# apache/paimon

Measured on NVIDIA H100. Metric: merged rows/sec at 16 runs x 40M rows, higher is better.
Workload: dtype int64

## Files before the change

### paimon_b200/csrc/api.cu

```cuda
#include <algorithm>
#include <cstdlib>
#include <cstring>
#include <map>
#include <memory>
#include <mutex>
#include <queue>

#include "pg_internal.h"

namespace pg {

static thread_local std::string g_last_error;
void set_error(const std::string &msg) { g_last_error = msg; }
pg_status fail(pg_status code, const std::string &msg) {
    g_last_error = msg;
    return code;
}

static int g_device = -1;

struct Arena {
    unsigned char *base = nullptr;
    size_t cap = 0, top = 0;
    cudaError_t reserve(size_t bytes) {
        top = 0;
        if (bytes <= cap) return cudaSuccess;
        if (base) cudaFree(base);
        base = nullptr;
        cap = 0;
        cudaError_t e = cudaMalloc((void **)&base, bytes);
        if (e == cudaSuccess) cap = bytes;
        return e;
    }
    void *take(size_t bytes) {
        size_t a = align256(top);
        if (a + bytes > cap) return nullptr;
        top = a + bytes;
        return base + a;
    }
    void release() {
        if (base) cudaFree(base);
        base = nullptr;
        cap = top = 0;
    }
    ~Arena() { release(); }
};

struct Merge {
    std::shared_ptr<const Spec> spec;
    std::vector<std::shared_ptr<const Run>> runs;
    std::vector<std::weak_ptr<const Run>> bound;
    std::vector<int64_t> row0;
    int k = 0;
    int64_t n_in = 0;
    size_t desc_cap = 0;
    cudaStream_t stream = nullptr;
    cudaEvent_t ev[5] = {nullptr, nullptr, nullptr, nullptr, nullptr};
    std::vector<int64_t> varlen_bound;
    KeyDesc key{};
    SeqFields seq{};
    MergeFlags flags{};
    std::vector<ColDesc> cols;
    std::vector<int32_t> varlen_cols;
    std::vector<uint8_t> emit;
    void *d_desc = nullptr;
    const void **d_key_ptrs = nullptr;
    const int32_t **d_key_offs = nullptr;
    const int64_t **d_seq_ptrs = nullptr;
    const int8_t **d_kind_ptrs = nullptr;
    ColPtrs d_ptrs{};
    int64_t *d_run_rows = nullptr;
    ColDesc *d_cols = nullptr;
    int32_t *d_tile_counter = nullptr;
    int32_t *d_col_order = nullptr;
    int32_t *d_varlen_cols = nullptr;
    int n_passes = 0;
    const SeqGroups *d_groups = nullptr;
    bool has_group_aggs = false;
    pg_out_column *d_out_cols = nullptr;
    int64_t *d_totals = nullptr;
    int32_t *d_err = nullptr;
    int64_t *h_totals = nullptr;
    int32_t *h_err = nullptr;
    std::vector<pg_out_column> out_cols;
    Arena work;
    Arena outbuf;
    int64_t n_out = 0;
    bool has_batch = false;
    pg_stats stats{};
    ~Merge() {
        if (g_device >= 0) cudaSetDevice(g_device);
        if (stream) cudaStreamSynchronize(stream);
        if (d_desc) cudaFree(d_desc);
        if (h_totals) cudaFreeHost(h_totals);
        for (cudaEvent_t e : ev) if (e) cudaEventDestroy(e);
        if (stream) cudaStreamDestroy(stream);
    }
};


Table<Schema> g_schemas(1);
static Table<Spec> g_specs(2);
Table<Run> g_runs(3);
static Table<Merge> g_merges(4);

pg_status ensure_device() {
    if (g_device < 0) return fail(PG_ERR_INVALID, "pg_init has not been called");
    PG_CUDA(cudaSetDevice(g_device));
    return PG_OK;
}

static pg_status copy_batch(std::vector<void *> &dsts, std::vector<void *> &srcs, std::vector<size_t> &sizes,
                            cudaMemcpyKind kind, cudaStream_t stream) {
    if (dsts.empty()) return PG_OK;
    static bool batch_ok = true;
    if (batch_ok && dsts.size() > 1) {
        cudaMemcpyAttributes attr{};
        attr.srcAccessOrder = cudaMemcpySrcAccessOrderStream;
        size_t attr_idx = 0, fail_idx = 0;
        cudaError_t e = cudaMemcpyBatchAsync(dsts.data(), srcs.data(), sizes.data(), dsts.size(), &attr, &attr_idx, 1,
                                             &fail_idx, stream);
        if (e == cudaSuccess) return PG_OK;
        cudaGetLastError();
        batch_ok = false;
    }
    for (size_t i = 0; i < dsts.size(); i++) PG_CUDA(cudaMemcpyAsync(dsts[i], srcs[i], sizes[i], kind, stream));
    return PG_OK;
}
static std::mutex g_buf_mu;
static std::multimap<size_t, void *> g_free_bufs;
static size_t g_free_bytes = 0;
static size_t buf_cache_limit() {
    static size_t lim = [] {
        const char *e = getenv("PG_RUN_CACHE_BYTES");
        return e ? (size_t)strtoull(e, nullptr, 10) : ((size_t)16 << 30);
    }();
    return lim;
}
static void buf_trim(size_t keep_bytes) {
    std::vector<void *> drop;
    {
        std::lock_guard<std::mutex> g(g_buf_mu);
        while (g_free_bytes > keep_bytes && !g_free_bufs.empty()) {
            auto it = std::prev(g_free_bufs.end());
            drop.push_back(it->second);
            g_free_bytes -= it->first;
            g_free_bufs.erase(it);
        }
    }
    for (void *p : drop) cudaFree(p);
}
void *buf_take(size_t bytes, size_t *got) {
    {
        std::lock_guard<std::mutex> g(g_buf_mu);
        auto it = g_free_bufs.lower_bound(bytes);
        if (it != g_free_bufs.end() && it->first <= bytes + bytes / 2 + (1 << 20)) {
            void *p = it->second;
            *got = it->first;
            g_free_bytes -= it->first;
            g_free_bufs.erase(it);
            return p;
        }
    }
    void *p = nullptr;
    if (cudaMalloc(&p, bytes) != cudaSuccess) {
        cudaGetLastError();
        buf_trim(0);
        if (cudaMalloc(&p, bytes) != cudaSuccess) return nullptr;
    }
    *got = bytes;
    return p;
}
void buf_give(void *p, size_t bytes) {
    {
        std::lock_guard<std::mutex> g(g_buf_mu);
        if (g_free_bytes + bytes <= buf_cache_limit()) {
            g_free_bufs.emplace(bytes, p);
            g_free_bytes += bytes;
            return;
        }
    }
    cudaFree(p);
}
cudaStream_t copy_stream() {
    static thread_local cudaStream_t st = nullptr;
    if (!st) cudaStreamCreateWithFlags(&st, cudaStreamNonBlocking);
    return st;
}

pg_status batch_columns(uint64_t handle, BatchColumns *out) {
    if (std::shared_ptr<Merge> m = g_merges.get(handle)) {
        if (!m->has_batch) return fail(PG_ERR_INVALID, "no batch: call pg_merge_execute first");
        if (m->stream) PG_CUDA(cudaStreamSynchronize(m->stream));
        out->schema = m->spec->schema;
        out->n_rows = m->n_out;
        for (const pg_out_column &oc : m->out_cols) out->cols.push_back(DevColumn{oc.data, oc.offsets, oc.validity});
        out->merge = std::move(m);
        return PG_OK;
    }
    std::shared_ptr<Run> r = g_runs.get(handle);
    if (!r) return fail(PG_ERR_INVALID, "unknown run / merge handle");
    out->schema = r->schema;
    out->n_rows = r->n_rows;
    out->cols = r->cols;
    out->run = std::move(r);
    return PG_OK;
}


pg_status oom(const char *who, const char *what, size_t bytes) {
    size_t fr = 0, tot = 0;
    cudaMemGetInfo(&fr, &tot);
    cudaGetLastError();
    return fail(PG_ERR_CUDA, std::string(who) + ": out of device memory for " + what + " (" + std::to_string(bytes >> 20) +
                                 " MiB wanted, " + std::to_string(fr >> 20) + " of " + std::to_string(tot >> 20) + " MiB free)");
}

pg_status check_file_desc(const pg_file_desc &f) {
    if (f.mem != PG_MEM_HOST && f.mem != PG_MEM_DEVICE)
        return fail(PG_ERR_INVALID, "file descriptor: memory kind " + std::to_string(f.mem) + " is neither host nor device");
    if (f.size < 0) return fail(PG_ERR_INVALID, "file descriptor: negative size");
    if (f.size > 0 && !f.bytes) return fail(PG_ERR_INVALID, "file descriptor: no bytes for a file of " + std::to_string(f.size) + " bytes");
    return PG_OK;
}

pg_status check_section_args(uint64_t schema, const pg_file_desc *files, int n_files, int n_runs, const uint64_t *out_runs,
                             std::shared_ptr<const Schema> *s) {
    *s = g_schemas.get(schema);
    if (!*s || !out_runs || n_files < 0 || n_runs < 0 || (n_files > 0 && !files))
        return fail(PG_ERR_INVALID, "bad schema handle or null argument");
    for (int i = 0; i < n_files; i++) {
        pg_status st = check_file_desc(files[i]);
        if (st) return st;
        if (files[i].run < 0 || files[i].run >= n_runs)
            return fail(PG_ERR_INVALID, "file descriptor: run index " + std::to_string(files[i].run) + " out of range");
    }
    return PG_OK;
}

pg_status file_image(Scratch &scratch, const uint8_t *bytes, int64_t size, const char *who, const uint8_t **out) {
    uint8_t *d = (uint8_t *)scratch.take((size_t)size + 64);
    if (!d) return oom(who, "a file image", (size_t)size);
    PG_CUDA(cudaMemcpyAsync(d, bytes, (size_t)size, cudaMemcpyHostToDevice, scratch.stream));
    *out = d;
    return PG_OK;
}

pg_status RunBuilder::read_columns(const uint8_t *read_cols, const char *const *column_names) {
    names = column_names;
    if (names)
        for (int c = 0; c < nc; c++)
            if (!names[c]) return fail(PG_ERR_INVALID, std::string(who) + ": column name " + std::to_string(c) + " is NULL");
    if (!read_cols) return PG_OK;
    for (int c = 0; c < schema->n_key + 2; c++)
        if (!read_cols[c]) return fail(PG_ERR_INVALID, std::string(who) + ": key, sequence number and kind columns are always read");
    for (int c = 0; c < nc; c++) read[c] = read_cols[c] != 0;
    return PG_OK;
}

pg_status RunBuilder::add_file(int run, int64_t rows, const std::vector<std::string> &cols) {
    if (!names && (int)cols.size() != nc)
        return fail(PG_ERR_UNSUPPORTED, std::string(who) + ": the file has " + std::to_string(cols.size()) + " columns and the "
                                        "read schema " + std::to_string(nc) + " (pass the field names)");
    std::unordered_map<std::string, int> by_name;
    if (names) for (int i = 0; i < (int)cols.size(); i++) by_name.emplace(cols[i], i);
    std::vector<int> fc(nc, -2);
    for (int c = 0; c < nc; c++) {
        if (!read[c]) continue;
        fc[c] = c;
        if (names) {
            auto it = by_name.find(names[c]);
            fc[c] = it == by_name.end() ? -1 : it->second;
        }
        if (fc[c] == -1 && (c < schema->n_key + 2 || !schema->field(c).nullable))
            return fail(PG_ERR_UNSUPPORTED, std::string(who) + ": the file has no column '" + names[c] + "' and the read "
                                            "schema does not allow NULL for it");
        const size_t i = (size_t)run * nc + c;
        if (fc[c] == -1) missing[i] = 1;
        if (rows > 0) with_rows[i] |= fc[c] == -1 ? 2 : 1;
    }
    file_col.push_back(std::move(fc));
    file_row0.push_back(place_file(run, rows));
    return PG_OK;
}

pg_status RunBuilder::check_runs() const {
    for (int64_t n : run_rows)
        if (n > 0x7fffffffLL) return fail(PG_ERR_UNSUPPORTED, std::string(who) + ": more than 2^31 rows in one run");
    for (size_t i = 0; i < with_rows.size(); i++)
        if (with_rows[i] == 3 && is_varlen(schema->field((int)(i % nc)).type))
            return fail(PG_ERR_UNSUPPORTED, std::string(who) + ": a var-len column exists in some files with rows of a sorted "
                                            "run only (mixed table schemas inside one run: not decoded on device)");
    return PG_OK;
}

pg_status RunBuilder::alloc(const std::vector<uint8_t> &bitmap, const std::vector<uint8_t> &zero) {
    const int n_runs = (int)run_rows.size();
    scratch.runs.resize(n_runs);
    out.assign((size_t)n_runs * nc, OutColumn());
    for (int r = 0; r < n_runs; r++) {
        const int64_t n = run_rows[r];
        scratch.runs[r] = std::make_unique<Run>(schema, n);
        auto main_bytes = [&](int c) { const int w = type_width(schema->field(c).type); return w ? (size_t)n * w : 4 * (size_t)(n + 1); };
        const size_t vb = align256((size_t)((n + 31) / 32) * 4 + 64);
        size_t vbytes = 0;
        for (int c = 0; c < nc; c++) if (read[c] && bitmap[c]) vbytes += vb;
        size_t total = vbytes;
        std::vector<size_t> o_main(nc);
        for (int c = 0; c < nc; c++) {
            o_main[c] = total;
            if (read[c]) total += align256(main_bytes(c) + 64);
        }
        scratch.runs[r]->bufs.emplace_back(total + 256);
        unsigned char *base = scratch.runs[r]->bufs.back().get();
        if (!base) return oom(who, "the columns of a run", total);
        if (vbytes) PG_CUDA(cudaMemsetAsync(base, 0, vbytes, scratch.stream));
        size_t vt = 0;
        for (int c = 0; c < nc; c++) {
            if (!read[c]) continue;
            OutColumn &o = out[(size_t)r * nc + c];
            if (bitmap[c]) { o.validity = (uint32_t *)(base + vt); vt += vb; decoded_bytes += (n + 7) / 8; }
            if (type_width(schema->field(c).type)) o.data = base + o_main[c];
            else o.offsets = (int32_t *)(base + o_main[c]);
            decoded_bytes += (int64_t)main_bytes(c);
            if (zero[(size_t)r * nc + c]) PG_CUDA(cudaMemsetAsync(base + o_main[c], 0, main_bytes(c), scratch.stream));
        }
    }
    return PG_OK;
}

pg_status RunBuilder::alloc_payload(const std::vector<int64_t> &payload) {
    bool any = false;
    for (int c = 0; c < nc; c++) any |= read[c] && is_varlen(schema->field(c).type);
    if (!any) return PG_OK;
    for (int r = 0; r < (int)run_rows.size(); r++) {
        size_t sum = 256;
        for (int c = 0; c < nc; c++)
            if (read[c] && is_varlen(schema->field(c).type)) sum += align256((size_t)payload[(size_t)r * nc + c] + 64);
        Run &run = *scratch.runs[r];
        run.bufs.emplace_back(sum);
        unsigned char *pl = run.bufs.back().get();
        if (!pl) return oom(who, "the var-len payload of a run", sum);
        size_t pt = 0;
        for (int c = 0; c < nc; c++) {
            if (!read[c] || !is_varlen(schema->field(c).type)) continue;
            const int64_t bytes = payload[(size_t)r * nc + c];
            out[(size_t)r * nc + c].data = pl + pt;
            run.varlen_bytes[c] = bytes;
            decoded_bytes += bytes;
            pt += align256((size_t)bytes + 64);
        }
    }
    return PG_OK;
}

void RunBuilder::finish(uint64_t *out_runs, int64_t bytes_h2d, pg_section_info *info) {
    const int n_runs = (int)run_rows.size();
    for (int r = 0; r < n_runs; r++) {
        Run &run = *scratch.runs[r];
        for (int c = 0; c < nc; c++) {
            const OutColumn &o = out[(size_t)r * nc + c];
            if (read[c]) run.cols[c] = DevColumn{o.data ? o.data : run.bufs[0].get(), o.offsets, (const uint8_t *)o.validity};
        }
        run.bytes_h2d = r == 0 ? bytes_h2d : 0;
        out_runs[r] = g_runs.put(std::move(scratch.runs[r]));
    }
    if (info) {
        memset(info, 0, sizeof(*info));
        for (int64_t n : run_rows) info->n_rows += n;
        info->n_runs = n_runs;
        info->decoded_bytes = decoded_bytes;
    }
}

SectionFrame::SectionFrame(std::shared_ptr<const Schema> s, int n_runs, const char *who)
    : stream(copy_stream()), scratch(stream), b(std::move(s), n_runs, scratch, who) {}

pg_status SectionFrame::start(const uint8_t *read_cols, const char *const *names) {
    PG_CUDA(cudaEventCreate(&tm.e0));
    PG_CUDA(cudaEventCreate(&tm.e1));
    PG_CUDA(cudaEventRecord(tm.e0, stream));
    return b.read_columns(read_cols, names);
}

pg_status SectionFrame::place(const pg_file_desc *files, int n_files) {
    d_file.assign(n_files, nullptr);
    for (int f = 0; f < n_files; f++) {
        file_bytes += files[f].size;
        if (files[f].mem == PG_MEM_DEVICE) { d_file[f] = files[f].bytes; continue; }
        { pg_status st = file_image(scratch, files[f].bytes, files[f].size, b.who, &d_file[f]); if (st) return st; }
        h2d += files[f].size;
    }
    return PG_OK;
}

pg_status SectionFrame::finish(const int32_t *d_err, uint64_t *out_runs, pg_section_info *info) {
    PG_CUDA(cudaEventRecord(tm.e1, stream));
    int32_t herr = 0;
    SmallReads rb(stream);
    { pg_status rs = rb.add(&herr, d_err, 4); if (!rs) rs = rb.finish(); if (rs) return rs; }
    PG_CUDA(cudaGetLastError());
    { pg_status st = kernel_error(herr, b.who); if (st) return st; }
    b.finish(out_runs, h2d, info);
    if (info) {
        info->file_bytes = file_bytes;
        info->page_bytes = page_bytes;
        info->n_files = (int32_t)d_file.size();
        info->launches = launches;
        info->ms_decode = tm.ms();
    }
    return PG_OK;
}

static void free_outputs(Merge *m, bool release_memory = false) {
    m->out_cols.clear();
    m->has_batch = false;
    if (release_memory) {
        if (m->stream) cudaStreamSynchronize(m->stream);
        m->outbuf.release();
    }
}


static bool agg_supports_retract(int agg) {
    return agg == PG_AGG_SUM || agg == PG_AGG_PRODUCT || agg == PG_AGG_LAST_VALUE ||
           agg == PG_AGG_LAST_NON_NULL_VALUE || agg == PG_AGG_PRIMARY_KEY;
}

static pg_status build_descriptors(Merge *m) {
    const Schema *s = m->spec->schema.get();
    const Spec *sp = m->spec.get();
    if (s->n_key < 1 || s->n_key > PG_MAX_KEY_FIELDS)
        return fail(PG_ERR_UNSUPPORTED, "more than 4 primary-key fields are not implemented on the device");
    m->key = KeyDesc{};
    m->key.n_fields = s->n_key;
    int key_bytes = 0;
    bool all_fixed = true;
    for (int f = 0; f < s->n_key; f++) {
        int t = s->key_fields[f].type;
        if (t == PG_FLOAT || t == PG_DOUBLE)
            return fail(PG_ERR_UNSUPPORTED, "FLOAT / DOUBLE primary keys are not implemented on the device "
                                            "(the reference's comparator treats NaN as equal to everything)");
        m->key.type[f] = t;
        m->key.width[f] = type_width(t);
        if (is_varlen(t)) all_fixed = false;
        key_bytes += type_width(t);
    }
    m->key.exact = all_fixed && key_bytes <= 8;
    m->seq = SeqFields{};
    if (sp->seq_fields.size() > 4)
        return fail(PG_ERR_UNSUPPORTED, "more than 4 'sequence.field' columns are not implemented on the device");
    for (size_t i = 0; i < sp->seq_fields.size(); i++) {
        int vf = sp->seq_fields[i];
        if (vf < 0 || vf >= s->n_val) return fail(PG_ERR_INVALID, "sequence.field index out of range");
        int t = s->val_fields[vf].type;
        if (is_varlen(t))
            return fail(PG_ERR_UNSUPPORTED, "var-len 'sequence.field' columns are not implemented on the device");
        m->seq.col[i] = s->n_key + 2 + vf;
        m->seq.type[i] = t;
        m->seq.width[i] = type_width(t);
    }
    m->seq.n = (int32_t)sp->seq_fields.size();
    m->seq.ascending = sp->seq_ascending ? 1 : 0;
    m->flags = MergeFlags{sp->engine, sp->ignore_delete, sp->remove_record_on_delete, sp->drop_delete};

    const int nc = s->n_cols();
    m->cols.assign(nc, ColDesc{});
    m->varlen_cols.clear();
    m->emit.assign(nc, 1);
    for (int c = s->n_key + 2; c < nc; c++)
        if (!sp->read_fields.empty() && !sp->read_fields[c - s->n_key - 2]) m->emit[c] = 0;
    std::vector<uint8_t> needed = m->emit;
    for (int32_t vf : sp->seq_fields) if (vf >= 0 && vf < s->n_val) needed[s->n_key + 2 + vf] = 1;
    for (int32_t vf : sp->group_seq_fields) if (vf >= 0 && vf < s->n_val) needed[s->n_key + 2 + vf] = 1;
    for (int r = 0; r < m->k; r++)
        for (int c = 0; c < nc; c++)
            if (needed[c] && m->runs[r]->n_rows > 0 && !m->runs[r]->cols[c].data && !m->runs[r]->cols[c].offsets)
                return fail(PG_ERR_INVALID, "run " + std::to_string(r) + " has no buffers for column " + std::to_string(c) +
                                            ", which the merge reads (read-type projection dropped a field the merge "
                                            "function compares or emits)");
    for (int c = 0; c < nc; c++) {
        pg_field f = s->field(c);
        ColDesc &cd = m->cols[c];
        cd.type = f.type;
        cd.width = type_width(f.type);
        cd.nullable = f.nullable;
        cd.agg = PG_AGG_NONE;
        cd.retract = RT_OK;
        cd.varlen_index = -1;
        cd.decimal = 0;
        if (is_varlen(f.type) && m->emit[c]) {
            cd.varlen_index = (int)m->varlen_cols.size();
            m->varlen_cols.push_back(c);
        }
        if (c < s->n_key) { cd.mode = CM_KEY; cd.nullable = 0; }
        else if (c == s->n_key) { cd.mode = CM_SEQ; cd.nullable = 0; }
        else if (c == s->n_key + 1) { cd.mode = CM_KIND; cd.nullable = 0; }
        else {
            int vi = c - s->n_key - 2;
            int agg = sp->agg.empty() ? PG_AGG_NONE : sp->agg[vi];
            bool ign = !sp->ignore_retract.empty() && sp->ignore_retract[vi];
            const int32_t dec = sp->decimal.empty() ? 0 : sp->decimal[vi];
            const int32_t fold_dec = agg == PG_AGG_SUM || agg == PG_AGG_PRODUCT ? dec : 0;
            if (sp->engine == PG_ENGINE_AGGREGATE) {
                if (agg == PG_AGG_NONE) agg = PG_AGG_LAST_NON_NULL_VALUE;
                bool numeric = f.type == PG_INT8 || f.type == PG_INT16 || f.type == PG_INT32 ||
                               f.type == PG_INT64 || f.type == PG_FLOAT || f.type == PG_DOUBLE;
                if ((agg == PG_AGG_SUM || agg == PG_AGG_PRODUCT) && !numeric)
                    return fail(PG_ERR_INVALID, "sum/product need a numeric column");
                if ((agg == PG_AGG_BOOL_AND || agg == PG_AGG_BOOL_OR) && f.type != PG_BOOL)
                    return fail(PG_ERR_INVALID, "bool_and/bool_or need a BOOLEAN column");
                if ((agg == PG_AGG_MAX || agg == PG_AGG_MIN) && f.type == PG_BOOL)
                    return fail(PG_ERR_INVALID, "Incomparable type: BOOLEAN");
                if (agg < PG_AGG_SUM || agg > PG_AGG_PRIMARY_KEY)
                    return fail(PG_ERR_UNSUPPORTED, "aggregate function not implemented on the device");
                cd.mode = CM_FOLD;
                cd.agg = agg;
                cd.decimal = fold_dec;
                cd.nullable = 1;
                cd.retract = ign ? RT_IGNORE : (agg_supports_retract(agg) ? RT_OK : RT_ERROR);
            } else {
                const bool in_group = sp->n_groups() > 0 && sp->field_group[vi] >= 0;
                if (sp->engine == PG_ENGINE_PARTIAL_UPDATE && !in_group && agg != PG_AGG_NONE &&
                    agg != PG_AGG_LAST_NON_NULL_VALUE && agg != PG_AGG_PRIMARY_KEY)
                    return fail(PG_ERR_INVALID, "Must use sequence group for aggregation functions");
                cd.mode = CM_SELECT;
                if (sp->n_groups() > 0 && sp->field_group[vi] >= 0) {
                    const int g = sp->field_group[vi];
                    bool is_seq = false;
                    for (int j = sp->group_seq_start[g]; j < sp->group_seq_start[g + 1]; j++)
                        if (sp->group_seq_fields[j] == vi) is_seq = true;
                    cd.mode = is_seq ? CM_GSEQ : CM_GVAL;
                    cd.agg = g;
                    cd.nullable = 1;
                    if (!is_seq && agg != PG_AGG_NONE) {
                        cd.mode = CM_GAGG;
                        cd.agg = agg;
                        cd.decimal = fold_dec;
                        cd.group = g;
                        cd.retract = ign ? RT_IGNORE : (agg_supports_retract(agg) ? RT_OK : RT_ERROR);
                        m->has_group_aggs = true;
                    }
                }
            }
        }
    }

    const int k = m->k, nk = s->n_key, nv = (int)m->varlen_cols.size();
    size_t o_key = 0;
    size_t o_koff = o_key + align256(sizeof(void *) * k * nk);
    size_t o_seq = o_koff + align256(sizeof(void *) * k * nk);
    size_t o_kind = o_seq + align256(sizeof(void *) * k);
    size_t o_pd = o_kind + align256(sizeof(void *) * k);
    size_t o_po = o_pd + align256(sizeof(void *) * (size_t)k * nc);
    size_t o_pv = o_po + align256(sizeof(void *) * (size_t)k * nc);
    size_t o_rows = o_pv + align256(sizeof(void *) * (size_t)k * nc);
    size_t o_cols = o_rows + align256(sizeof(int64_t) * k);
    size_t o_out = o_cols + align256(sizeof(ColDesc) * nc);
    size_t o_tot = o_out + align256(sizeof(pg_out_column) * nc);
    size_t o_err = o_tot + align256(sizeof(int64_t) * (nv + 1));
    size_t o_cnt = o_err + 256;
    size_t o_ord = o_cnt + 256;
    size_t o_vlc = o_ord + align256(sizeof(int32_t) * (2 * (size_t)nc + 2));
    size_t o_sg = o_vlc + align256(sizeof(int32_t) * (size_t)(nv + 1));
    size_t total = o_sg + align256(sizeof(SeqGroups));
    std::vector<unsigned char> host(total, 0);
    m->varlen_bound.assign(nv, 0);
    for (int r = 0; r < k; r++) {
        const Run *run = m->runs[r].get();
        for (int f = 0; f < nk; f++) {
            ((const void **)(host.data() + o_key))[r * nk + f] = run->cols[f].data;
            ((const void **)(host.data() + o_koff))[r * nk + f] = run->cols[f].offsets;
        }
        ((const void **)(host.data() + o_seq))[r] = run->cols[nk].data;
        ((const void **)(host.data() + o_kind))[r] = run->cols[nk + 1].data;
        for (int c = 0; c < nc; c++) {
            ((const void **)(host.data() + o_pd))[(size_t)c * k + r] = run->cols[c].data;
            ((const void **)(host.data() + o_po))[(size_t)c * k + r] = run->cols[c].offsets;
            ((const void **)(host.data() + o_pv))[(size_t)c * k + r] = run->cols[c].validity;
            if (m->cols[c].varlen_index >= 0) m->varlen_bound[m->cols[c].varlen_index] += run->varlen_bytes[c];
        }
        ((int64_t *)(host.data() + o_rows))[r] = run->n_rows;
    }
    memcpy(host.data() + o_cols, m->cols.data(), sizeof(ColDesc) * nc);
    {
        int32_t *ord = (int32_t *)(host.data() + o_ord);
        int32_t *vlc = (int32_t *)(host.data() + o_vlc);
        int n = 0;
        for (int c = 0; c < nc; c++) if (m->emit[c] && m->cols[c].width == 0) ord[n++] = c;
        for (int c = 0; c < nc; c++) if (m->emit[c] && m->cols[c].width != 0) ord[n++] = c;
        m->n_passes = n;
        for (int v = 0; v < nv; v++) vlc[v] = m->varlen_cols[v];
    }
    m->d_groups = nullptr;
    if (sp->n_groups() > 0) {
        SeqGroups *sg = (SeqGroups *)(host.data() + o_sg);
        sg->n = sp->n_groups();
        for (int g = 0; g <= sg->n; g++) sg->start[g] = sp->group_seq_start[g];
        for (int j = 0; j < sp->group_seq_start[sg->n]; j++) {
            const int vf = sp->group_seq_fields[j];
            sg->col[j] = s->n_key + 2 + vf;
            sg->type[j] = s->val_fields[vf].type;
            sg->width[j] = type_width(s->val_fields[vf].type);
        }
        for (int g = 0; g < sg->n; g++) sg->partial_delete[g] = sp->group_partial_delete[g];
    }
    if (!m->d_desc || total > m->desc_cap) {
        if (m->d_desc) cudaFree(m->d_desc);
        m->d_desc = nullptr;
        PG_CUDA(cudaMalloc(&m->d_desc, total));
        m->desc_cap = total;
    }
    { pg_status ts = small_h2d(m->d_desc, host.data(), total, m->stream); if (ts) return ts; }
    PG_CUDA(cudaStreamSynchronize(m->stream));
    unsigned char *d = (unsigned char *)m->d_desc;
    m->d_key_ptrs = (const void **)(d + o_key);
    m->d_key_offs = (const int32_t **)(d + o_koff);
    m->d_seq_ptrs = (const int64_t **)(d + o_seq);
    m->d_kind_ptrs = (const int8_t **)(d + o_kind);
    m->d_ptrs.data = (const void *const *)(d + o_pd);
    m->d_ptrs.offsets = (const int32_t *const *)(d + o_po);
    m->d_ptrs.validity = (const uint32_t *const *)(d + o_pv);
    m->d_run_rows = (int64_t *)(d + o_rows);
    m->d_cols = (ColDesc *)(d + o_cols);
    m->d_out_cols = (pg_out_column *)(d + o_out);
    m->d_totals = (int64_t *)(d + o_tot);
    m->d_err = (int32_t *)(d + o_err);
    m->d_tile_counter = (int32_t *)(d + o_cnt);
    m->d_col_order = (int32_t *)(d + o_ord);
    m->d_varlen_cols = (int32_t *)(d + o_vlc);
    if (sp->n_groups() > 0) m->d_groups = (const SeqGroups *)(d + o_sg);
    if (!m->h_totals) PG_CUDA(cudaMallocHost((void **)&m->h_totals, sizeof(int64_t) * (nv + 1) + 16));
    m->h_err = (int32_t *)(m->h_totals + nv + 1);
    return PG_OK;
}

pg_status kernel_error(int code, const char *who) {
    static const struct { int code; pg_status st; const char *msg; } kErrors[] = {
        {KERR_PU_DELETE, PG_ERR_MERGE_FUNCTION,
         "By default, Partial update can not accept delete records, you can choose one of the "
         "following solutions:\n1. Configure 'ignore-delete' to ignore delete records.\n"
         "2. Configure 'partial-update.remove-record-on-delete' to remove the whole row when "
         "receiving delete records.\n3. Configure 'sequence-group's to retract partial columns. "
         "Also configure 'partial-update.remove-record-on-sequence-group' to remove the whole "
         "row when receiving deleted records of `specified sequence group`."},
        {KERR_FIRST_ROW_RETRACT, PG_ERR_MERGE_FUNCTION,
         "By default, First row merge engine can not accept DELETE/UPDATE_BEFORE records.\n"
         "You can config 'ignore-delete' to ignore the DELETE/UPDATE_BEFORE records."},
        {KERR_AGG_RETRACT, PG_ERR_MERGE_FUNCTION,
         "Aggregate function does not support retraction, If you allow this function to ignore "
         "retraction messages, you can configure 'fields.${field_name}.ignore-retract'='true'."},
        {KERR_DIV_ZERO, PG_ERR_MERGE_FUNCTION, "ArithmeticException: / by zero"},
        {KERR_DEC_DIV_ZERO, PG_ERR_MERGE_FUNCTION, "ArithmeticException: Division by zero"},
        {KERR_DEC_DIV_UNDEFINED, PG_ERR_MERGE_FUNCTION, "ArithmeticException: Division undefined"},
        {KERR_DEC_NON_TERMINATING, PG_ERR_MERGE_FUNCTION,
         "ArithmeticException: Non-terminating decimal expansion; no exact representable decimal result."},
        {KERR_TILE_OVERFLOW, PG_ERR_INTERNAL,
         "a merge tile overflowed (does a run contain duplicate keys? SortMergeReader.java:37 requires unique keys per reader)"},
        {KERR_OFFSET_OVERFLOW, PG_ERR_INTERNAL, "a var-len column exceeds 2 GiB of payload"},
        {KERR_BAD_PAGE, PG_ERR_FORMAT, "a page or stream does not decode (malformed file or unsupported encoding)"},
        {KERR_PQ_HEADER, PG_ERR_FORMAT, "malformed or truncated page header"},
        {KERR_PQ_NO_DICT, PG_ERR_FORMAT, "dictionary-encoded page without dictionary"},
        {KERR_PQ_ROWS, PG_ERR_FORMAT, "page row counts do not add up"},
        {KERR_PQ_DICT_ID, PG_ERR_FORMAT, "dictionary id outside the dictionary"},
        {KERR_PQ_ENCODING, PG_ERR_UNSUPPORTED,
         "a page uses a value encoding the device decoder does not implement (PLAIN, dictionary, DELTA_BINARY_PACKED "
         "integers and RLE booleans are decoded)"},
        {KERR_PQ_LEVELS, PG_ERR_UNSUPPORTED, "repetition levels / BIT_PACKED definition levels are not decoded on device"},
    };
    if (code == KERR_NONE) return PG_OK;
    for (const auto &e : kErrors)
        if (e.code == code) return fail(e.st, e.st == PG_ERR_MERGE_FUNCTION ? std::string(e.msg) : std::string(who) + ": " + e.msg);
    return fail(PG_ERR_INTERNAL, std::string(who) + ": unknown kernel error " + std::to_string(code));
}


static pg_status execute(Merge *m) {
    pg_status st = ensure_device();
    if (st) return st;
    cudaStream_t sm = m->stream;
    free_outputs(m);
    for (size_t r = m->runs.size(); r < m->bound.size(); r++)
        if (!m->runs.emplace_back(m->bound[r].lock())) {
            m->runs.clear();
            return fail(PG_ERR_INVALID, "a run of this merge has been freed since it was merged: rebind first");
        }
    const Schema *s = m->spec->schema.get();
    const int k = m->k, nc = s->n_cols(), nv = (int)m->varlen_cols.size();
    m->stats = pg_stats{};
    m->stats.rows_in = m->n_in;
    int launches = 0;

    const int S = kSampleStride;
    const int q = kPlanTile / S - 2 * k;
    if (q < 1) return fail(PG_ERR_UNSUPPORTED, "too many runs for one merge call");
    std::vector<LevelView> views;
    std::vector<int64_t> level_total;
    {
        int64_t stride = 1;
        while (true) {
            LevelView lv{};
            lv.stride = stride;
            int64_t tot = 0;
            for (int r = 0; r < k; r++) {
                lv.row0[r] = m->row0[r];
                lv.count[r] = (m->runs[r]->n_rows - m->row0[r]) / stride;
                tot += lv.count[r];
            }
            views.push_back(lv);
            level_total.push_back(tot);
            if (tot <= kPlanTile) break;
            stride *= S;
        }
    }
    const int top = (int)views.size() - 1;
    std::vector<int> n_tiles(top + 1);
    n_tiles[top] = 1;
    for (int l = top - 1; l >= 0; l--) n_tiles[l] = (int)((level_total[l + 1] + q - 1) / q);
    m->stats.n_levels = top;
    m->stats.n_tiles = n_tiles[0];

    PG_CUDA(cudaMemsetAsync(m->d_err, 0, sizeof(int32_t), sm));
    PG_CUDA(cudaEventRecord(m->ev[0], sm));

    MergeLaunch ml{k, m->key, KeySrc{m->d_key_ptrs, m->d_key_offs}, sm, m->d_err, nullptr};
    {
        size_t need = 4096;
        auto add = [&](size_t b) { need += align256(b ? b : 16); };
        for (int l = top; l >= 0; l--) {
            add(sizeof(int64_t) * (size_t)(n_tiles[l] + 1) * k);
            if (l > 0) { add(sizeof(uint64_t) * (size_t)std::max<int64_t>(level_total[l], 1)); add(sizeof(uint64_t) * (size_t)std::max<int64_t>(level_total[l], 1)); }
        }
        int64_t skipped = 0;
        for (int r = 0; r < k; r++) skipped += m->row0[r];
        const size_t N_ = (size_t)(m->n_in + skipped), T_ = (size_t)n_tiles[0];
        add(2 * N_ + 16); add(m->d_groups ? 4 * N_ + 16 : 16); add(m->has_group_aggs ? 4 * N_ + 16 : 16); add(4 * T_); add(8 * N_ + 16); add(N_ + 16); add(8 * T_); add(8 * T_ * std::max(nv, 1));
        PG_CUDA(m->work.reserve(need));
    }
    auto talloc = [&](size_t bytes, void **out) -> cudaError_t {
        *out = m->work.take(bytes ? bytes : 16);
        return *out ? cudaSuccess : cudaErrorMemoryAllocation;
    };

    if (!m->key.exact) {
        int *d_skip = nullptr;
        PG_CUDA(talloc(sizeof(int), (void **)&d_skip));
        launch_key_lcp(ml, views[0], d_skip);
        ml.skip = d_skip;
        launches++;
    }
    int64_t *bounds0 = nullptr;
    uint64_t *sk_above = nullptr;
    uint64_t *sref_above = nullptr;
    for (int l = top; l >= 0; l--) {
        int64_t *bounds = nullptr;
        PG_CUDA(talloc(sizeof(int64_t) * (size_t)(n_tiles[l] + 1) * k, (void **)&bounds));
        launch_partition(ml, views[l], sk_above, sref_above, q, n_tiles[l], bounds);
        launches++;
        if (l > 0) {
            uint64_t *sk = nullptr;
            PG_CUDA(talloc(sizeof(uint64_t) * (size_t)std::max<int64_t>(level_total[l], 1), (void **)&sk));
            uint64_t *sref = nullptr;
            PG_CUDA(talloc(sizeof(uint64_t) * (size_t)std::max<int64_t>(level_total[l], 1), (void **)&sref));
            launch_merge_keys(ml, views[l], bounds, n_tiles[l], sk, sref);
            sref_above = sref;
            launches++;
            sk_above = sk;
        } else {
            bounds0 = bounds;
        }
    }
    PG_CUDA(cudaEventRecord(m->ev[1], sm));

    const int T = n_tiles[0];
    int64_t N = m->n_in;
    for (int r = 0; r < k; r++) N += m->row0[r];
    uint16_t *plan = nullptr;
    int32_t *tile_rows = nullptr;
    int64_t *tmp_seq = nullptr, *row_base = nullptr;
    uint64_t *vl_state = nullptr;
    int8_t *tmp_kind = nullptr;
    PG_CUDA(talloc(sizeof(uint16_t) * (size_t)N + 16, (void **)&plan));
    uint32_t *gplan = nullptr;
    if (m->d_groups) PG_CUDA(talloc(sizeof(uint32_t) * (size_t)N + 16, (void **)&gplan));
    uint32_t *gagg = nullptr;
    if (m->has_group_aggs) PG_CUDA(talloc(sizeof(uint32_t) * (size_t)N + 16, (void **)&gagg));
    PG_CUDA(talloc(sizeof(int32_t) * (size_t)T, (void **)&tile_rows));
    PG_CUDA(talloc(sizeof(int64_t) * (size_t)N + 16, (void **)&tmp_seq));
    PG_CUDA(talloc((size_t)N + 16, (void **)&tmp_kind));
    PG_CUDA(talloc(sizeof(int64_t) * (size_t)T, (void **)&row_base));
    PG_CUDA(talloc(sizeof(uint64_t) * (size_t)T * std::max(nv, 1), (void **)&vl_state));
    PG_CUDA(cudaMemsetAsync(vl_state, 0, sizeof(uint64_t) * (size_t)T * std::max(nv, 1), sm));
    PG_CUDA(cudaMemsetAsync(m->d_tile_counter, 0, sizeof(int32_t), sm));

    PlanArgs pa{};
    pa.bounds = bounds0;
    pa.n_tiles = T;
    pa.seq_ptrs = m->d_seq_ptrs;
    pa.kind_ptrs = m->d_kind_ptrs;
    pa.flags = m->flags;
    pa.seq = m->seq;
    pa.ptrs = m->d_ptrs;
    pa.plan = plan;
    pa.tile_rows = tile_rows;
    pa.tmp_seq = tmp_seq;
    pa.tmp_kind = tmp_kind;
    pa.groups = m->d_groups;
    pa.gplan = gplan;
    pa.gagg = gagg;
    launch_plan(ml, pa);
    launch_scan(sm, tile_rows, T, row_base, m->d_totals);
    launches += 2;
    PG_CUDA(cudaEventRecord(m->ev[2], sm));
    {
        SmallReads rb(sm);
        pg_status rs = rb.add(m->h_totals, m->d_totals, sizeof(int64_t));
        if (!rs) rs = rb.add(m->h_err, m->d_err, sizeof(int32_t));
        if (!rs) rs = rb.finish();
        if (rs) return rs;
    }
    if (*m->h_err != KERR_NONE) return kernel_error(*m->h_err, "merge");

    const int64_t n_out = m->h_totals[0];
    m->n_out = n_out;
    m->out_cols.assign(nc, pg_out_column{});
    int64_t bytes_out = 0;
    {
        size_t need = 4096, vbytes = 0;
        for (int c = 0; c < nc; c++) {
            const ColDesc &cd = m->cols[c];
            if (!m->emit[c]) continue;
            if (cd.nullable) vbytes += align256((size_t)((n_out + 31) / 32) * 4 + 64);
            if (cd.width > 0) need += align256((size_t)n_out * cd.width + 64);
            else need += align256((size_t)m->varlen_bound[cd.varlen_index] + 64) + align256(4 * (size_t)(n_out + 1) + 64);
        }
        if (nv > 0) need += align256(sizeof(uint16_t) * (size_t)nv * (size_t)(n_out + 64) + 64);
        PG_CUDA(m->outbuf.reserve(need + vbytes));
        if (vbytes) {
            void *v0 = m->outbuf.take(vbytes);
            PG_CUDA(cudaMemsetAsync(v0, 0, vbytes, sm));
            m->outbuf.top = 0;
        }
    }
    auto oalloc = [&](size_t bytes, void **out) -> cudaError_t {
        *out = m->outbuf.take(bytes);
        return *out ? cudaSuccess : cudaErrorMemoryAllocation;
    };
    for (int c = 0; c < nc; c++) {
        if (m->cols[c].nullable && m->emit[c]) {
            size_t vb = (size_t)((n_out + 31) / 32) * 4 + 64;
            PG_CUDA(oalloc(vb, (void **)&m->out_cols[c].validity));
            bytes_out += (n_out + 7) / 8;
        }
    }
    for (int c = 0; c < nc; c++) {
        const ColDesc &cd = m->cols[c];
        pg_out_column &oc = m->out_cols[c];
        if (!m->emit[c]) continue;
        if (cd.width > 0) {
            oc.data_bytes = n_out * cd.width;
            PG_CUDA(oalloc((size_t)oc.data_bytes + 64, &oc.data));
        } else {
            oc.data_bytes = m->varlen_bound[cd.varlen_index];
            PG_CUDA(oalloc((size_t)oc.data_bytes + 64, &oc.data));
            PG_CUDA(oalloc(sizeof(int32_t) * (size_t)(n_out + 1) + 64, (void **)&oc.offsets));
            bytes_out += 4 * (n_out + 1);
        }
        if (cd.width > 0) bytes_out += oc.data_bytes;
    }
    m->stats.bytes_out = bytes_out;
    { pg_status ts = small_h2d(m->d_out_cols, m->out_cols.data(), sizeof(pg_out_column) * nc, sm); if (ts) return ts; }

    EmitArgs ea{};
    ea.bounds = bounds0;
    ea.n_tiles = (T + 1) / 2;
    ea.n_plan_tiles = T;
    ea.tile_rows = tile_rows;
    ea.k = k;
    ea.plan = plan;
    ea.row_base = row_base;
    ea.tmp_seq = tmp_seq;
    ea.tmp_kind = tmp_kind;
    ea.gplan = gplan;
    ea.gagg = gagg;
    ea.cols = m->d_cols;
    ea.col_order = m->d_col_order;
    ea.n_passes = m->n_passes;
    ea.varlen_cols = m->d_varlen_cols;
    ea.ptrs = m->d_ptrs;
    ea.run_rows = m->d_run_rows;
    ea.n_cols = nc;
    ea.n_varlen = nv;
    ea.out_cols = m->d_out_cols;
    ea.totals = m->d_totals;
    ea.vl_state = vl_state;
    ea.tile_counter = m->d_tile_counter;
    ea.err = m->d_err;
    ea.stream = sm;
    PG_CUDA(cudaEventRecord(m->ev[4], sm));
    launch_emit(ea);
    launches++;
    PG_CUDA(cudaEventRecord(m->ev[3], sm));
    {
        SmallReads rb(sm);
        pg_status rs = rb.add(m->h_err, m->d_err, sizeof(int32_t));
        if (!rs) rs = rb.add(m->h_totals, m->d_totals, sizeof(int64_t) * (nv + 1));
        if (!rs) rs = rb.finish();
        if (rs) return rs;
    }
    PG_CUDA(cudaGetLastError());
    m->has_batch = true;
    if (*m->h_err != KERR_NONE) {
        free_outputs(m);
        return kernel_error(*m->h_err, "merge");
    }
    for (int c = 0; c < nc; c++)
        if (m->cols[c].width == 0 && m->emit[c]) {
            m->out_cols[c].data_bytes = m->h_totals[1 + m->cols[c].varlen_index];
            m->stats.bytes_out += m->out_cols[c].data_bytes;
        }
    m->stats.rows_out = n_out;
    m->stats.launches = launches;
    cudaEventElapsedTime(&m->stats.ms_partition, m->ev[0], m->ev[1]);
    cudaEventElapsedTime(&m->stats.ms_plan, m->ev[1], m->ev[2]);
    cudaEventElapsedTime(&m->stats.ms_alloc, m->ev[2], m->ev[4]);
    cudaEventElapsedTime(&m->stats.ms_emit, m->ev[4], m->ev[3]);
    cudaEventElapsedTime(&m->stats.ms_total, m->ev[0], m->ev[3]);
    m->runs.clear();
    return PG_OK;
}

}


using namespace pg;

extern "C" {

const char *pg_last_error(void) { return g_last_error.c_str(); }
int32_t pg_abi_version(void) { return PG_ABI_VERSION; }

pg_status pg_init(int32_t device_ordinal) {
    int n = 0;
    cudaError_t e = cudaGetDeviceCount(&n);
    if (e != cudaSuccess || n == 0)
        return fail(PG_ERR_CUDA, std::string("no CUDA device: libpaimon_gpu has no CPU fallback (") +
                                     cudaGetErrorString(e) + ")");
    if (device_ordinal < 0 || device_ordinal >= n) return fail(PG_ERR_INVALID, "bad device ordinal");
    if (g_device >= 0 && g_device != device_ordinal)
        return fail(PG_ERR_INVALID, "pg_init: this process is already bound to device " + std::to_string(g_device) +
                                    " (one process per GPU: handles, streams and cached buffers belong to it)");
    PG_CUDA(cudaSetDevice(device_ordinal));
    g_device = device_ordinal;
    cudaMemPool_t pool;
    PG_CUDA(cudaDeviceGetDefaultMemPool(&pool, device_ordinal));
    uint64_t thr = UINT64_MAX;
    PG_CUDA(cudaMemPoolSetAttribute(pool, cudaMemPoolAttrReleaseThreshold, &thr));
    return PG_OK;
}

pg_status pg_shutdown(void) {
    if (g_device >= 0) {
        cudaSetDevice(g_device);
        cudaDeviceSynchronize();
        buf_trim(0);
        cudaMemPool_t pool;
        if (cudaDeviceGetDefaultMemPool(&pool, g_device) == cudaSuccess) cudaMemPoolTrimTo(pool, 0);
    }
    return PG_OK;
}

pg_status pg_schema_create(const pg_schema_desc *desc, uint64_t *out_schema) {
    if (!desc || !out_schema) return fail(PG_ERR_INVALID, "null argument");
    if (desc->n_key < 1 || desc->n_val < 0 || desc->n_key + 2 + desc->n_val > kMaxCols)
        return fail(PG_ERR_INVALID, "bad field counts");
    auto s = std::make_unique<Schema>();
    s->n_key = desc->n_key;
    s->n_val = desc->n_val;
    for (int i = 0; i < desc->n_key; i++) {
        if (!type_ok(desc->key_fields[i].type)) return fail(PG_ERR_INVALID, "bad key field type");
        s->key_fields.push_back(pg_field{desc->key_fields[i].type, 0});
    }
    for (int i = 0; i < desc->n_val; i++) {
        if (!type_ok(desc->val_fields[i].type)) return fail(PG_ERR_INVALID, "bad value field type");
        s->val_fields.push_back(desc->val_fields[i]);
    }
    *out_schema = g_schemas.put(std::move(s));
    return PG_OK;
}

pg_status pg_schema_info(uint64_t schema, int32_t *n_key, int32_t *n_val) {
    std::shared_ptr<Schema> s = g_schemas.get(schema);
    if (!s) return fail(PG_ERR_INVALID, "unknown schema handle");
    if (n_key) *n_key = s->n_key;
    if (n_val) *n_val = s->n_val;
    return PG_OK;
}

pg_status pg_schema_free(uint64_t schema) {
    return g_schemas.take(schema) ? PG_OK : fail(PG_ERR_INVALID, "unknown schema handle");
}

pg_status pg_merge_spec_create(uint64_t schema, const pg_merge_spec *spec, uint64_t *out_spec) {
    std::shared_ptr<Schema> s = g_schemas.get(schema);
    if (!s || !spec || !out_spec) return fail(PG_ERR_INVALID, "bad schema handle or null argument");
    if (spec->engine < PG_ENGINE_DEDUPLICATE || spec->engine > PG_ENGINE_FIRST_ROW)
        return fail(PG_ERR_INVALID, "Unsupported merge engine");
    if (spec->n_sequence_groups < 0 || (spec->n_sequence_groups > 0 && (!spec->group_seq_start ||
                                                                         !spec->group_seq_fields || !spec->field_group)))
        return fail(PG_ERR_INVALID, "bad sequence group description");
    if (spec->n_sequence_groups > 0 && spec->engine != PG_ENGINE_PARTIAL_UPDATE)
        return fail(PG_ERR_INVALID, "sequence groups belong to the partial-update merge engine");
    if (spec->n_sequence_groups > PG_MAX_SEQ_GROUPS)
        return fail(PG_ERR_UNSUPPORTED, "more than 16 sequence groups are not implemented on the device");
    auto sp = std::make_unique<Spec>();
    sp->schema = s;
    sp->engine = spec->engine;
    sp->ignore_delete = spec->ignore_delete != 0;
    sp->remove_record_on_delete = spec->remove_record_on_delete != 0;
    sp->drop_delete = spec->drop_delete != 0;
    sp->seq_ascending = spec->seq_ascending;
    if (spec->n_seq_fields < 0 || (spec->n_seq_fields > 0 && !spec->seq_fields))
        return fail(PG_ERR_INVALID, "bad sequence.field description");
    for (int i = 0; i < spec->n_seq_fields; i++) {
        if (spec->seq_fields[i] < 0 || spec->seq_fields[i] >= s->n_val) return fail(PG_ERR_INVALID, "sequence.field index out of range");
        sp->seq_fields.push_back(spec->seq_fields[i]);
    }
    if (spec->agg) sp->agg.assign(spec->agg, spec->agg + s->n_val);
    if (spec->ignore_retract) sp->ignore_retract.assign(spec->ignore_retract, spec->ignore_retract + s->n_val);
    if (spec->read_fields) sp->read_fields.assign(spec->read_fields, spec->read_fields + s->n_val);
    if (spec->decimal) {
        sp->decimal.assign(spec->decimal, spec->decimal + s->n_val);
        for (int f = 0; f < s->n_val; f++) {
            const int32_t d = sp->decimal[f];
            if (d == 0) continue;
            const int p = d >> 8, sc = d & 0xff;
            if (p > 18)
                return fail(PG_ERR_UNSUPPORTED, "DECIMAL(p > 18) is not implemented on the device (field " +
                                                    std::to_string(f) + ")");
            if (p < 1 || sc > p || s->val_fields[f].type != PG_INT64)
                return fail(PG_ERR_INVALID, "bad DECIMAL description of value field " + std::to_string(f) +
                                                " (precision 1..18, scale <= precision, an INT64 column)");
        }
    }
    if (spec->n_sequence_groups > 0) {
        const int ng = spec->n_sequence_groups;
        sp->group_seq_start.assign(spec->group_seq_start, spec->group_seq_start + ng + 1);
        sp->group_seq_fields.assign(spec->group_seq_fields, spec->group_seq_fields + sp->group_seq_start[ng]);
        sp->field_group.assign(spec->field_group, spec->field_group + s->n_val);
        sp->group_partial_delete.assign(ng, 0);
        for (int g = 0; g < ng; g++) {
            const int n = sp->group_seq_start[g + 1] - sp->group_seq_start[g];
            if (n < 1) return fail(PG_ERR_INVALID, "a sequence group needs a sequence field");
            if (n > 4)
                return fail(PG_ERR_UNSUPPORTED, "more than 4 sequence fields in one sequence group are not "
                                                "implemented on the device");
            for (int j = sp->group_seq_start[g]; j < sp->group_seq_start[g + 1]; j++) {
                const int f = sp->group_seq_fields[j];
                if (f < 0 || f >= s->n_val) return fail(PG_ERR_INVALID, "sequence group field out of range");
                if (is_varlen(s->val_fields[f].type))
                    return fail(PG_ERR_UNSUPPORTED, "var-len sequence-group fields are not implemented on the device");
                if (spec->group_partial_delete && spec->group_partial_delete[f]) sp->group_partial_delete[g] = 1;
            }
        }
        for (int f = 0; f < s->n_val; f++) {
            if (sp->field_group[f] < -1 || sp->field_group[f] >= ng)
                return fail(PG_ERR_INVALID, "field_group out of range");
            if (sp->field_group[f] >= 0 && !sp->agg.empty() && sp->agg[f] != PG_AGG_NONE) {
                const int agg = sp->agg[f], t = s->val_fields[f].type;
                if (is_varlen(t))
                    return fail(PG_ERR_UNSUPPORTED, "aggregate functions on var-len fields inside a sequence group "
                                                    "are not implemented on the device");
                if (agg < PG_AGG_SUM || agg > PG_AGG_PRIMARY_KEY)
                    return fail(PG_ERR_UNSUPPORTED, "aggregate function not implemented on the device");
                const bool numeric = t == PG_INT8 || t == PG_INT16 || t == PG_INT32 || t == PG_INT64 ||
                                     t == PG_FLOAT || t == PG_DOUBLE;
                if ((agg == PG_AGG_SUM || agg == PG_AGG_PRODUCT) && !numeric)
                    return fail(PG_ERR_INVALID, "sum/product need a numeric column");
                if ((agg == PG_AGG_BOOL_AND || agg == PG_AGG_BOOL_OR) && t != PG_BOOL)
                    return fail(PG_ERR_INVALID, "bool_and/bool_or need a BOOLEAN column");
            }
        }
    }
    if (sp->engine == PG_ENGINE_PARTIAL_UPDATE && sp->ignore_delete && sp->remove_record_on_delete)
        return fail(PG_ERR_INVALID, "ignore-delete and partial-update.remove-record-on-delete have conflicting "
                                    "behavior so should not be enabled at the same time.");
    *out_spec = g_specs.put(std::move(sp));
    return PG_OK;
}

pg_status pg_merge_spec_free(uint64_t spec) {
    return g_specs.take(spec) ? PG_OK : fail(PG_ERR_INVALID, "unknown spec handle");
}

pg_status pg_trim(void) {
    buf_trim(0);
    return PG_OK;
}

pg_status pg_run_open(uint64_t schema, const pg_run_desc *desc, int32_t mem, uint64_t *out_run) {
    std::shared_ptr<Schema> s = g_schemas.get(schema);
    if (!s || !desc || !out_run) return fail(PG_ERR_INVALID, "bad schema handle or null argument");
    if (desc->n_rows < 0 || desc->n_rows > 0x7fffffffLL) return fail(PG_ERR_INVALID, "bad row count");
    pg_status st = ensure_device();
    if (st) return st;
    auto run = std::make_unique<Run>(s, desc->n_rows);
    const int nc = s->n_cols();
    const int64_t n = desc->n_rows;
    if (mem == PG_MEM_DEVICE) {
        for (int c = 0; c < nc; c++) {
            const pg_column &pc = desc->cols[c];
            if ((((uintptr_t)pc.data) | ((uintptr_t)pc.offsets) | ((uintptr_t)pc.validity)) & 15)
                return fail(PG_ERR_INVALID, "device column buffers must be 16-byte aligned");
            run->cols[c] = DevColumn{pc.data, pc.offsets, pc.validity};
            if (is_varlen(s->field(c).type) && n > 0) {
                if (!pc.offsets) return fail(PG_ERR_INVALID, "var-len column without offsets");
                int32_t last = 0;
                PG_CUDA(cudaMemcpy(&last, pc.offsets + n, sizeof(int32_t), cudaMemcpyDeviceToHost));
                run->varlen_bytes[c] = last;
            }
        }
    } else if (mem == PG_MEM_HOST) {
        std::vector<size_t> o_data(nc), o_off(nc), o_val(nc), b_data(nc), b_off(nc), b_val(nc);
        size_t total = 0;
        for (int c = 0; c < nc; c++) {
            pg_field f = s->field(c);
            const pg_column &pc = desc->cols[c];
            if (is_varlen(f.type)) {
                if (n > 0 && !pc.offsets) return fail(PG_ERR_INVALID, "var-len column without offsets");
                b_off[c] = sizeof(int32_t) * (size_t)(n + 1);
                if (n > 0 && pc.offsets[n] < pc.offsets[0]) return fail(PG_ERR_INVALID, "decreasing offsets");
                b_data[c] = n > 0 ? (size_t)(pc.offsets[n] - pc.offsets[0]) : 0;
                run->varlen_base[c] = n > 0 ? pc.offsets[0] : 0;
            } else {
                b_off[c] = 0;
                b_data[c] = (size_t)n * type_width(f.type);
            }
            b_val[c] = pc.validity ? (size_t)((n + 7) / 8) : 0;
            o_data[c] = total; total += align256(b_data[c] + 16);
            o_off[c] = total; total += align256(b_off[c]);
            o_val[c] = total; total += align256(b_val[c] + 8);
        }
        cudaStream_t cs = copy_stream();
        Scratch scratch(cs);
        unsigned char *d = (unsigned char *)scratch.take(total + 256);
        if (!d) return fail(PG_ERR_CUDA, "out of device memory for a run");
        std::vector<void *> cp_dst, cp_src;
        std::vector<size_t> cp_size;
        auto add_copy = [&](void *dst, const void *src, size_t bytes) {
            cp_dst.push_back(dst); cp_src.push_back(const_cast<void *>(src)); cp_size.push_back(bytes);
        };
        for (int c = 0; c < nc; c++) {
            const pg_column &pc = desc->cols[c];
            DevColumn dc;
            dc.data = d + o_data[c] - run->varlen_base[c];
            if (b_data[c]) add_copy(d + o_data[c], (const unsigned char *)pc.data + run->varlen_base[c], b_data[c]);
            if (b_off[c]) {
                dc.offsets = (const int32_t *)(d + o_off[c]);
                if (n >= 0 && pc.offsets) add_copy(d + o_off[c], pc.offsets, b_off[c]);
            }
            if (b_val[c]) {
                dc.validity = d + o_val[c];
                add_copy(d + o_val[c], pc.validity, b_val[c]);
            }
            run->bytes_h2d += (int64_t)(b_data[c] + b_off[c] + b_val[c]);
            if (is_varlen(s->field(c).type)) run->varlen_bytes[c] = (int64_t)b_data[c];
            run->cols[c] = dc;
        }
        pg_status cst = copy_batch(cp_dst, cp_src, cp_size, cudaMemcpyHostToDevice, cs);
        if (cst) return cst;
        PG_CUDA(cudaStreamSynchronize(cs));
        run->bufs.swap(scratch.bufs);
    } else {
        return fail(PG_ERR_INVALID, "bad memory kind");
    }
    *out_run = g_runs.put(std::move(run));
    return PG_OK;
}

pg_status pg_run_free(uint64_t run) {
    return g_runs.take(run) ? PG_OK : fail(PG_ERR_INVALID, "unknown run handle");
}

pg_status pg_run_layout(uint64_t run, int64_t *n_rows, int64_t *data_bytes, int32_t *has_validity, int32_t n_cols) {
    std::shared_ptr<Run> r = g_runs.get(run);
    if (!r || !n_rows) return fail(PG_ERR_INVALID, "unknown run handle");
    const int nc = r->schema->n_cols();
    if (n_cols != nc) return fail(PG_ERR_INVALID, "column count mismatch");
    *n_rows = r->n_rows;
    for (int c = 0; c < nc; c++) {
        pg_field f = r->schema->field(c);
        const bool absent = !r->cols[c].data && !r->cols[c].offsets;
        if (data_bytes) data_bytes[c] = absent ? -1 : (is_varlen(f.type) ? r->varlen_bytes[c] : r->n_rows * type_width(f.type));
        if (has_validity) has_validity[c] = r->cols[c].validity != nullptr;
    }
    return PG_OK;
}

pg_status pg_run_fetch(uint64_t run, const pg_out_column *host_cols, int32_t n_cols) {
    std::shared_ptr<Run> r = g_runs.get(run);
    if (!r || !host_cols) return fail(PG_ERR_INVALID, "unknown run handle");
    const int nc = r->schema->n_cols();
    if (n_cols != nc) return fail(PG_ERR_INVALID, "column count mismatch");
    pg_status st = ensure_device();
    if (st) return st;
    const int64_t n = r->n_rows;
    for (int c = 0; c < nc && n > 0; c++) {
        pg_field f = r->schema->field(c);
        const DevColumn &dc = r->cols[c];
        const pg_out_column &hc = host_cols[c];
        size_t db = is_varlen(f.type) ? (size_t)r->varlen_bytes[c] : (size_t)n * type_width(f.type);
        if (!dc.data && !dc.offsets) continue;
        if (db && hc.data && (size_t)hc.data_bytes < db)
            return fail(PG_ERR_INVALID, "pg_run_fetch: data buffer of column " + std::to_string(c) + " is too small");
        if (db && hc.data)
            PG_CUDA(cudaMemcpy(hc.data, (const unsigned char *)dc.data + (c < (int)r->varlen_base.size() ? r->varlen_base[c] : 0),
                               db, cudaMemcpyDeviceToHost));
        if (dc.offsets && hc.offsets)
            PG_CUDA(cudaMemcpy(hc.offsets, dc.offsets, sizeof(int32_t) * (size_t)(n + 1), cudaMemcpyDeviceToHost));
        if (dc.validity && hc.validity)
            PG_CUDA(cudaMemcpy(hc.validity, dc.validity, (size_t)((n + 7) / 8), cudaMemcpyDeviceToHost));
    }
    return PG_OK;
}

}

static pg_status make_slice(uint64_t source, int64_t row_lo, int64_t row_hi, uint64_t *out_run, int64_t *start_row) {
    BatchColumns batch;
    pg_status st = batch_columns(source, &batch);
    if (st) return st;
    if (row_lo < 0 || row_hi < row_lo || row_hi > batch.n_rows) return fail(PG_ERR_INVALID, "slice outside the source");
    const int64_t lo = row_lo & ~(int64_t)127;
    auto run = std::make_unique<Run>(batch.schema, row_hi - lo);
    run->source = batch.run;
    const int nc = batch.schema->n_cols();
    for (int c = 0; c < nc; c++) {
        const pg_field f = batch.schema->field(c);
        DevColumn dc = batch.cols[c];
        if (is_varlen(f.type)) {
            if (dc.offsets && run->n_rows > 0) {
                int32_t b[2] = {0, 0};
                PG_CUDA(cudaMemcpy(&b[0], dc.offsets + lo, 4, cudaMemcpyDeviceToHost));
                PG_CUDA(cudaMemcpy(&b[1], dc.offsets + row_hi, 4, cudaMemcpyDeviceToHost));
                run->varlen_base[c] = b[0];
                run->varlen_bytes[c] = b[1] - b[0];
            }
            if (dc.offsets) dc.offsets += lo;
        } else if (dc.data) {
            dc.data = (const unsigned char *)dc.data + lo * type_width(f.type);
        }
        if (dc.validity) dc.validity += lo / 8;
        run->cols[c] = dc;
    }
    if (start_row) *start_row = row_lo - lo;
    *out_run = g_runs.put(std::move(run));
    return PG_OK;
}

extern "C" {

pg_status pg_run_slice(uint64_t source, int64_t row_lo, int64_t row_hi, uint64_t *out_run, int64_t *start_row) {
    if (!out_run) return fail(PG_ERR_INVALID, "null argument");
    pg_status st = ensure_device();
    if (st) return st;
    return make_slice(source, row_lo, row_hi, out_run, start_row);
}

pg_status pg_thread_stream(void **out_cuda_stream) {
    if (!out_cuda_stream) return fail(PG_ERR_INVALID, "null argument");
    pg_status st = ensure_device();
    if (st) return st;
    *out_cuda_stream = (void *)copy_stream();
    return PG_OK;
}

static pg_status bind_runs(Merge *m, const uint64_t *runs, int32_t k, const int64_t *row0) {
    const Spec *sp = m->spec.get();
    m->runs.clear();
    m->bound.clear();
    m->row0.clear();
    m->k = 0;
    m->n_in = 0;
    m->stats = pg_stats{};
    for (int i = 0; i < k; i++) {
        std::shared_ptr<Run> r = g_runs.get(runs[i]);
        if (!r) return fail(PG_ERR_INVALID, "unknown run handle");
        if (r->schema != sp->schema) {
            const Schema *a = r->schema.get(), *b = sp->schema.get();
            bool same = a->n_key == b->n_key && a->n_val == b->n_val;
            for (int c = 0; same && c < a->n_cols(); c++)
                same = a->field(c).type == b->field(c).type && a->field(c).nullable == b->field(c).nullable;
            if (!same) return fail(PG_ERR_INVALID, "run and spec use different schemas");
        }
        const int64_t skip = row0 ? row0[i] : 0;
        if (skip < 0 || skip > r->n_rows) return fail(PG_ERR_INVALID, "start row outside the run");
        m->stats.bytes_h2d += r->bytes_h2d;
        if (r->n_rows - skip == 0) continue;
        m->runs.push_back(r);
        m->bound.push_back(r);
        m->row0.push_back(skip);
        m->n_in += r->n_rows - skip;
    }
    m->k = (int)m->runs.size();
    pg_status st = m->k > 0 ? build_descriptors(m) : PG_OK;
    if (st) m->k = 0;
    return st;
}

pg_status pg_merge_open(uint64_t spec, const uint64_t *runs, int32_t k, uint64_t *out_merge) {
    std::shared_ptr<Spec> sp = g_specs.get(spec);
    if (!sp || !out_merge || (k > 0 && !runs)) return fail(PG_ERR_INVALID, "bad spec handle or null argument");
    if (k < 0) return fail(PG_ERR_INVALID, "negative run count");
    if (k > PG_MAX_RUNS)
        return fail(PG_ERR_UNSUPPORTED, "more than PG_MAX_RUNS runs in one merge call");
    pg_status st = ensure_device();
    if (st) return st;
    std::unique_ptr<Merge> m(new Merge());
    m->spec = std::move(sp);
    PG_CUDA(cudaStreamCreateWithFlags(&m->stream, cudaStreamNonBlocking));
    for (auto &e : m->ev) PG_CUDA(cudaEventCreate(&e));
    st = bind_runs(m.get(), runs, k, nullptr);
    if (st) return st;
    *out_merge = g_merges.put(std::move(m));
    return PG_OK;
}

pg_status pg_merge_rebind(uint64_t merge, const uint64_t *runs, int32_t k, const int64_t *start_rows) {
    std::shared_ptr<Merge> m = g_merges.get(merge);
    if (!m || (k > 0 && !runs)) return fail(PG_ERR_INVALID, "unknown merge handle or null argument");
    if (k < 0 || k > PG_MAX_RUNS) return fail(PG_ERR_INVALID, "bad run count");
    pg_status st = ensure_device();
    if (st) return st;
    PG_CUDA(cudaStreamSynchronize(m->stream));
    free_outputs(m.get());
    return bind_runs(m.get(), runs, k, start_rows);
}

pg_status pg_merge_execute(uint64_t merge) {
    std::shared_ptr<Merge> m = g_merges.get(merge);
    if (!m) return fail(PG_ERR_INVALID, "unknown merge handle");
    if (m->k == 0 || m->n_in == 0) {
        free_outputs(m.get());
        m->n_out = 0;
        m->out_cols.assign(m->spec->schema->n_cols(), pg_out_column{});
        m->has_batch = true;
        m->stats = pg_stats{};
        return PG_OK;
    }
    int64_t h2d = m->stats.bytes_h2d;
    pg_status st = execute(m.get());
    m->stats.bytes_h2d = h2d;
    return st;
}

pg_status pg_merge_device_batch(uint64_t merge, pg_batch *out) {
    std::shared_ptr<Merge> m = g_merges.get(merge);
    if (!m || !out) return fail(PG_ERR_INVALID, "unknown merge handle");
    if (!m->has_batch) return fail(PG_ERR_INVALID, "no batch: call pg_merge_execute first");
    out->n_rows = m->n_out;
    out->n_cols = (int32_t)m->out_cols.size();
    out->cols = m->out_cols.data();
    return PG_OK;
}

pg_status pg_merge_fetch(uint64_t merge, const pg_out_column *host_cols, int32_t n_cols) {
    std::shared_ptr<Merge> m = g_merges.get(merge);
    if (!m || !host_cols) return fail(PG_ERR_INVALID, "unknown merge handle");
    if (!m->has_batch) return fail(PG_ERR_INVALID, "no batch: call pg_merge_execute first");
    if (n_cols != (int32_t)m->out_cols.size()) return fail(PG_ERR_INVALID, "column count mismatch");
    pg_status st = ensure_device();
    if (st) return st;
    const int64_t n = m->n_out;
    int64_t bytes = 0;
    std::vector<void *> cp_dst, cp_src;
    std::vector<size_t> cp_size;
    for (int c = 0; c < n_cols && n > 0; c++) {
        const pg_out_column &oc = m->out_cols[c];
        const pg_out_column &hc = host_cols[c];
        if (oc.data_bytes && hc.data) {
            if (hc.data_bytes < oc.data_bytes)
                return fail(PG_ERR_INVALID, "pg_merge_fetch: data buffer of column " + std::to_string(c) + " holds " +
                                            std::to_string(hc.data_bytes) + " bytes, the batch needs " + std::to_string(oc.data_bytes));
            cp_dst.push_back(hc.data); cp_src.push_back(oc.data); cp_size.push_back((size_t)oc.data_bytes);
            bytes += oc.data_bytes;
        }
        if (oc.offsets && hc.offsets) {
            cp_dst.push_back(hc.offsets); cp_src.push_back(oc.offsets); cp_size.push_back(sizeof(int32_t) * (size_t)(n + 1));
            bytes += 4 * (n + 1);
        }
        if (oc.validity && hc.validity) {
            cp_dst.push_back(hc.validity); cp_src.push_back(oc.validity); cp_size.push_back((size_t)((n + 7) / 8));
            bytes += (n + 7) / 8;
        }
    }
    st = copy_batch(cp_dst, cp_src, cp_size, cudaMemcpyDeviceToHost, m->stream);
    if (st) return st;
    PG_CUDA(cudaStreamSynchronize(m->stream));
    m->stats.bytes_d2h = bytes;
    return PG_OK;
}

pg_status pg_merge_release(uint64_t merge) {
    std::shared_ptr<Merge> m = g_merges.get(merge);
    if (!m) return fail(PG_ERR_INVALID, "unknown merge handle");
    if (ensure_device() == PG_OK) free_outputs(m.get(), true);
    return PG_OK;
}

pg_status pg_merge_stats(uint64_t merge, pg_stats *out) {
    std::shared_ptr<Merge> m = g_merges.get(merge);
    if (!m || !out) return fail(PG_ERR_INVALID, "unknown merge handle");
    *out = m->stats;
    return PG_OK;
}

pg_status pg_merge_stream(uint64_t merge, void **out_cuda_stream) {
    std::shared_ptr<Merge> m = g_merges.get(merge);
    if (!m || !out_cuda_stream) return fail(PG_ERR_INVALID, "unknown merge handle");
    *out_cuda_stream = (void *)m->stream;
    return PG_OK;
}

pg_status pg_merge_free(uint64_t merge) {
    return g_merges.take(merge) ? PG_OK : fail(PG_ERR_INVALID, "unknown merge handle");
}

pg_status pg_interval_partition(int32_t n_files, const int64_t *min_key, const int64_t *max_key,
                                int32_t *section_of, int32_t *run_of, int32_t *n_sections) {
    if (n_files < 0 || (n_files > 0 && (!min_key || !max_key || !section_of || !run_of)) || !n_sections)
        return fail(PG_ERR_INVALID, "null argument");
    std::vector<int> order(n_files);
    for (int i = 0; i < n_files; i++) order[i] = i;
    std::stable_sort(order.begin(), order.end(), [&](int a, int b) {
        if (min_key[a] != min_key[b]) return min_key[a] < min_key[b];
        return max_key[a] < max_key[b];
    });
    int sections = 0;
    size_t begin = 0;
    auto close_section = [&](size_t b, size_t e) {
        using Item = std::pair<int64_t, int>;
        std::priority_queue<Item, std::vector<Item>, std::greater<Item>> heap;
        int n_runs = 0;
        for (size_t i = b; i < e; i++) {
            int f = order[i];
            if (!heap.empty() && min_key[f] > heap.top().first) {
                Item top = heap.top();
                heap.pop();
                run_of[f] = top.second;
                heap.push(Item(max_key[f], top.second));
            } else {
                run_of[f] = n_runs;
                heap.push(Item(max_key[f], n_runs++));
            }
            section_of[f] = sections;
        }
        sections++;
    };
    int64_t bound = 0;
    for (size_t i = 0; i < (size_t)n_files; i++) {
        int f = order[i];
        if (i > begin && min_key[f] > bound) {
            close_section(begin, i);
            begin = i;
        }
        if (i == begin || max_key[f] > bound) bound = max_key[f];
    }
    if ((size_t)n_files > begin) close_section(begin, n_files);
    *n_sections = sections;
    return PG_OK;
}

}
```

### paimon_b200/csrc/emit.cu

```cuda
#include <stdio.h>

#include "device_utils.cuh"

namespace pg {

constexpr int kStages = 2;
constexpr int kEmitThreads = 512;
constexpr int kEmitWarps = kEmitThreads / 32;
#define kFlagAgg (1ull << 62)
#define kFlagPrefix (2ull << 62)
#define kValMask ((1ull << 62) - 1)

constexpr uint32_t kPmPosMask = 0x1FFF;
constexpr int kPmOpShift = 13;
constexpr uint32_t kPmHead = 0x8000;

struct EmitLayout {
    int rt;
    size_t stage_bytes;
    size_t total;
};
__host__ __device__ inline EmitLayout emit_layout(int k) {
    EmitLayout L;
    L.rt = kTileMax + 64 * k;
    L.stage_bytes = (((size_t)L.rt * 8 + (size_t)L.rt / 32 * 4) + 127) & ~(size_t)127;
    L.total = kStages * L.stage_bytes + (size_t)kTileMax * (2 + 2 + 1) + (PG_MAX_RUNS + 1) * 4 * 3 +
              PG_MAX_RUNS * 8 + kStages * PG_MAX_RUNS * 8 + kStages * 8 + 34 * 4 + 64;
    return L;
}

__device__ __forceinline__ bool staged_valid(const uint32_t *vw, int p) { return (vw[p >> 5] >> (p & 31)) & 1; }

template <int W> __device__ __forceinline__ uint64_t lds_fixed(const unsigned char *vals, int p);
template <> __device__ __forceinline__ uint64_t lds_fixed<1>(const unsigned char *v, int p) { return v[p]; }
template <> __device__ __forceinline__ uint64_t lds_fixed<2>(const unsigned char *v, int p) { return ((const uint16_t *)v)[p]; }
template <> __device__ __forceinline__ uint64_t lds_fixed<4>(const unsigned char *v, int p) { return ((const uint32_t *)v)[p]; }
template <> __device__ __forceinline__ uint64_t lds_fixed<8>(const unsigned char *v, int p) { return ((const uint64_t *)v)[p]; }
template <typename T> __device__ __forceinline__ T *as_global(T *p) { __builtin_assume(__isGlobal(p)); return p; }
template <int W> __device__ __forceinline__ void stg_fixed(void *d, int64_t row, uint64_t v);
template <> __device__ __forceinline__ void stg_fixed<1>(void *d, int64_t r, uint64_t v) { as_global((uint8_t *)d)[r] = (uint8_t)v; }
template <> __device__ __forceinline__ void stg_fixed<2>(void *d, int64_t r, uint64_t v) { as_global((uint16_t *)d)[r] = (uint16_t)v; }
template <> __device__ __forceinline__ void stg_fixed<4>(void *d, int64_t r, uint64_t v) { as_global((uint32_t *)d)[r] = (uint32_t)v; }
template <> __device__ __forceinline__ void stg_fixed<8>(void *d, int64_t r, uint64_t v) { as_global((uint64_t *)d)[r] = v; }

template <bool GAGG>
__device__ __forceinline__ int select_pos(const uint16_t *pm, const uint32_t *vw, int last) {
    int j = last;
    while (true) {
        uint32_t e = pm[j];
        uint32_t op = (e >> kPmOpShift) & 3;
        if (GAGG && op == OP_RETRACT) op = (e & kPmHead) ? OP_SET : OP_NOOP;
        if (op != OP_NOOP) {
            int pj = e & kPmPosMask;
            if (staged_valid(vw, pj)) return pj;
            if (op == OP_SET) return -1;
        }
        if (e & kPmHead) return -1;
        --j;
    }
}
template <bool GAGG>
__device__ __forceinline__ int select_member_idx(const uint16_t *pm, const uint32_t *vw, int last) {
    int j = last;
    while (true) {
        uint32_t e = pm[j];
        uint32_t op = (e >> kPmOpShift) & 3;
        if (GAGG && op == OP_RETRACT) op = (e & kPmHead) ? OP_SET : OP_NOOP;
        if (op != OP_NOOP) {
            if (staged_valid(vw, e & kPmPosMask)) return j;
            if (op == OP_SET) return -1;
        }
        if (e & kPmHead) return -1;
        --j;
    }
}

__device__ __forceinline__ int select_marked_idx(const uint16_t *pm, const uint32_t *gplan, uint32_t bit, int last) {
    int j = last;
    while (true) {
        if (gplan[j] & bit) return j;
        if (pm[j] & kPmHead) return -1;
        --j;
    }
}

__device__ __forceinline__ int group_first(const uint16_t *pm, int last) {
    int j = last;
    while (!(pm[j] & kPmHead)) --j;
    return j;
}

__device__ int fold_member_idx(const ColDesc &cd, const uint16_t *pm, const uint8_t *mrun, const uint32_t *vw,
                               const int32_t *offs, const uint8_t *const *cdata, int last, int32_t *err) {
    int acc = -1;
    bool initialized = false;
    for (int j = group_first(pm, last); j <= last; j++) {
        uint32_t e = pm[j];
        int op = (e >> kPmOpShift) & 3;
        if (op == OP_NOOP) continue;
        bool v = staged_valid(vw, e & kPmPosMask);
        int in = v ? j : -1;
        if (op == OP_SET) { acc = in; continue; }
        if (op == OP_RETRACT) {
            if (cd.retract == RT_IGNORE) continue;
            switch (cd.agg) {
                case PG_AGG_LAST_VALUE: acc = -1; break;
                case PG_AGG_LAST_NON_NULL_VALUE: if (v) acc = -1; break;
                case PG_AGG_PRIMARY_KEY: acc = in; break;
                default: atomicCAS(err, KERR_NONE, KERR_AGG_RETRACT); break;
            }
            continue;
        }
        switch (cd.agg) {
            case PG_AGG_LAST_VALUE: case PG_AGG_PRIMARY_KEY: acc = in; break;
            case PG_AGG_LAST_NON_NULL_VALUE: if (v) acc = in; break;
            case PG_AGG_FIRST_VALUE: if (!initialized) { initialized = true; acc = in; } break;
            case PG_AGG_FIRST_NON_NULL_VALUE: if (!initialized && v) { initialized = true; acc = in; } break;
            case PG_AGG_MAX: case PG_AGG_MIN:
                if (acc < 0 || in < 0) { if (acc < 0) acc = in; break; }
                {
                    int pa = pm[acc] & kPmPosMask, pb = e & kPmPosMask;
                    int d = bytes_compare(cdata[mrun[acc]] + offs[pa], offs[pa + 1] - offs[pa],
                                          cdata[mrun[j]] + offs[pb], offs[pb + 1] - offs[pb]);
                    if (cd.agg == PG_AGG_MAX) { if (d < 0) acc = in; }
                    else { if (!(d < 0)) acc = in; }
                }
                break;
            default: break;
        }
    }
    return acc;
}

template <bool DEC>
__device__ __forceinline__ uint64_t fold_arith(const ColDesc &cd, int fn, uint64_t a, uint64_t b, bool *valid,
                                               int32_t *err) {
    if (DEC) {
        const DecimalResult d = decimal_arith(cd.decimal, fn, a, b, err);
        *valid = d.valid;
        return d.value;
    }
    *valid = true;
    return fn == 4 ? negate_fixed(cd.type, cd.width, a) : arith(cd.type, cd.width, fn, a, b, err);
}

template <bool DEC>
__device__ void fold_fixed(const ColDesc &cd, const uint16_t *pm, const uint32_t *vw, const unsigned char *vals,
                           int last, uint64_t *out_val, bool *out_valid, int32_t *err) {
    const int w = cd.width;
    uint64_t val = 0;
    bool is_valid = false, initialized = false;
    for (int j = group_first(pm, last); j <= last; j++) {
        uint32_t e = pm[j];
        int op = (e >> kPmOpShift) & 3;
        if (op == OP_NOOP) continue;
        int pj = e & kPmPosMask;
        bool v = staged_valid(vw, pj);
        uint64_t in = v ? load_fixed(vals, w, pj) : 0;
        if (op == OP_SET) { val = in; is_valid = v; continue; }
        if (op == OP_RETRACT) {
            if (cd.retract == RT_IGNORE) continue;
            switch (cd.agg) {
                case PG_AGG_SUM:
                    if (!is_valid) { if (v) val = fold_arith<DEC>(cd, 4, in, 0, &is_valid, err); }
                    else if (v) val = fold_arith<DEC>(cd, 1, val, in, &is_valid, err);
                    break;
                case PG_AGG_PRODUCT:
                    if (is_valid && v) val = fold_arith<DEC>(cd, 3, val, in, &is_valid, err);
                    break;
                case PG_AGG_LAST_VALUE: is_valid = false; val = 0; break;
                case PG_AGG_LAST_NON_NULL_VALUE: if (v) { is_valid = false; val = 0; } break;
                case PG_AGG_PRIMARY_KEY: val = in; is_valid = v; break;
                default: atomicCAS(err, KERR_NONE, KERR_AGG_RETRACT); break;
            }
            continue;
        }
        switch (cd.agg) {
            case PG_AGG_SUM: case PG_AGG_PRODUCT:
                if (!is_valid || !v) { if (!is_valid) { val = in; is_valid = v; } }
                else val = fold_arith<DEC>(cd, cd.agg == PG_AGG_SUM ? 0 : 2, val, in, &is_valid, err);
                break;
            case PG_AGG_MAX: case PG_AGG_MIN:
                if (!is_valid || !v) { if (!is_valid) { val = in; is_valid = v; } }
                else {
                    int d = compare_fixed(cd.type, w, val, in);
                    if (cd.agg == PG_AGG_MAX) { if (d < 0) val = in; }
                    else { if (!(d < 0)) val = in; }
                }
                break;
            case PG_AGG_BOOL_AND: case PG_AGG_BOOL_OR:
                if (!is_valid || !v) { if (!is_valid) { val = in; is_valid = v; } }
                else val = cd.agg == PG_AGG_BOOL_AND ? ((val != 0) && (in != 0)) : ((val != 0) || (in != 0));
                break;
            case PG_AGG_LAST_VALUE: case PG_AGG_PRIMARY_KEY: val = in; is_valid = v; break;
            case PG_AGG_LAST_NON_NULL_VALUE: if (v) { val = in; is_valid = true; } break;
            case PG_AGG_FIRST_VALUE:
                if (!initialized) { initialized = true; val = in; is_valid = v; }
                break;
            case PG_AGG_FIRST_NON_NULL_VALUE:
                if (!initialized && v) { initialized = true; val = in; is_valid = true; }
                break;
            default: break;
        }
    }
    *out_val = val;
    *out_valid = is_valid;
}

template <bool DEC>
__device__ void agg_pair(const ColDesc &cd, uint64_t a, bool av, uint64_t b, bool bv, bool *initialized,
                         uint64_t *out, bool *out_valid, int32_t *err) {
    const int w = cd.width;
    switch (cd.agg) {
        case PG_AGG_SUM: case PG_AGG_PRODUCT:
            if (!av || !bv) { *out = av ? a : b; *out_valid = av || bv; }
            else *out = fold_arith<DEC>(cd, cd.agg == PG_AGG_SUM ? 0 : 2, a, b, out_valid, err);
            return;
        case PG_AGG_MAX: case PG_AGG_MIN:
            if (!av || !bv) { *out = av ? a : b; *out_valid = av || bv; return; }
            {
                const int d = compare_fixed(cd.type, w, a, b);
                const bool take_b = cd.agg == PG_AGG_MAX ? d < 0 : !(d < 0);
                *out = take_b ? b : a; *out_valid = true;
            }
            return;
        case PG_AGG_BOOL_AND: case PG_AGG_BOOL_OR:
            if (!av || !bv) { *out = av ? a : b; *out_valid = av || bv; return; }
            *out = cd.agg == PG_AGG_BOOL_AND ? ((a != 0) && (b != 0)) : ((a != 0) || (b != 0));
            *out_valid = true;
            return;
        case PG_AGG_LAST_VALUE: case PG_AGG_PRIMARY_KEY: *out = b; *out_valid = bv; return;
        case PG_AGG_LAST_NON_NULL_VALUE: *out = bv ? b : a; *out_valid = bv ? true : av; return;
        case PG_AGG_FIRST_VALUE:
            if (!*initialized) { *initialized = true; *out = b; *out_valid = bv; }
            else { *out = a; *out_valid = av; }
            return;
        case PG_AGG_FIRST_NON_NULL_VALUE:
            if (!*initialized && bv) { *initialized = true; *out = b; *out_valid = true; }
            else { *out = a; *out_valid = av; }
            return;
        default: *out = a; *out_valid = av; return;
    }
}

template <bool DEC>
__device__ void fold_group_agg(const ColDesc &cd, const uint16_t *pm, const uint32_t *gagg, const uint32_t *vw,
                               const unsigned char *vals, int last, uint64_t *out_val, bool *out_valid, int32_t *err) {
    const int w = cd.width, g = cd.group;
    uint64_t val = 0;
    bool is_valid = false, initialized = false;
    for (int j = group_first(pm, last); j <= last; j++) {
        const uint32_t e = pm[j];
        const int op = (e >> kPmOpShift) & 3;
        if (op == OP_NOOP) continue;
        const int pj = e & kPmPosMask;
        const bool v = staged_valid(vw, pj);
        const uint64_t in = v ? load_fixed(vals, w, pj) : 0;
        if (op == OP_SET) { val = in; is_valid = v; continue; }
        const uint32_t marks = gagg[j];
        if (op == OP_RETRACT) {
            if (e & kPmHead) { val = in; is_valid = v; }
            if (!((marks >> g) & 1) || cd.retract == RT_IGNORE) continue;
            switch (cd.agg) {
                case PG_AGG_SUM:
                    if (!is_valid) { if (v) val = fold_arith<DEC>(cd, 4, in, 0, &is_valid, err); }
                    else if (v) val = fold_arith<DEC>(cd, 1, val, in, &is_valid, err);
                    break;
                case PG_AGG_PRODUCT:
                    if (is_valid && v) val = fold_arith<DEC>(cd, 3, val, in, &is_valid, err);
                    break;
                case PG_AGG_LAST_VALUE: is_valid = false; val = 0; break;
                case PG_AGG_LAST_NON_NULL_VALUE: if (v) { is_valid = false; val = 0; } break;
                case PG_AGG_PRIMARY_KEY: val = in; is_valid = v; break;
                default: atomicCAS(err, KERR_NONE, KERR_AGG_RETRACT); break;
            }
            continue;
        }
        uint64_t r;
        bool rv;
        if ((marks >> g) & 1) agg_pair<DEC>(cd, val, is_valid, in, v, &initialized, &r, &rv, err);
        else if ((marks >> (16 + g)) & 1) agg_pair<DEC>(cd, in, v, val, is_valid, &initialized, &r, &rv, err);
        else continue;
        val = rv ? r : 0;
        is_valid = rv;
    }
    *out_val = val;
    *out_valid = is_valid;
}

struct TileView {
    const uint16_t *pm;
    const uint16_t *glast;
    int n_out;
    int o_shift;
    int64_t out_base;
    int64_t in_base;
    int n_out_a;
    int seq_shift;
};
__device__ __forceinline__ int64_t result_index(const TileView &tv, int ob) {
    return tv.in_base + ob + (ob >= tv.n_out_a ? tv.seq_shift : 0);
}

__device__ __forceinline__ void put_validity_word(uint8_t *validity, int64_t out_base, int wb, int n_out,
                                                  bool bit) {
    unsigned mask = __ballot_sync(0xffffffffu, bit);
    if ((threadIdx.x & 31) == 0) {
        int64_t word = (out_base + wb) >> 5;
        bool full = wb >= 0 && wb + 32 <= n_out;
        uint32_t *bm = as_global((uint32_t *)validity);
        if (full) bm[word] = mask;
        else if (mask) atomicOr(&bm[word], mask);
    }
}

template <int W, bool GAGG>
__device__ __forceinline__ void emit_fixed_column(const EmitArgs &ea, const ColDesc &cd, const pg_out_column &oc,
                                                  const TileView &tv, const unsigned char *vals, const uint32_t *vw) {
    const int tid = threadIdx.x, lane = tid & 31;
    for (int wb = (tid & ~31) - tv.o_shift; wb < tv.n_out; wb += kEmitThreads) {
        const int ob = wb + lane;
        const bool active = ob >= 0 && ob < tv.n_out;
        bool is_valid = false;
        if (active) {
            uint64_t val = 0;
            const int last = tv.glast[ob];
            if (cd.mode == CM_SELECT) {
                int pj = select_pos<GAGG>(tv.pm, vw, last);
                if (pj >= 0) { val = lds_fixed<W>(vals, pj); is_valid = true; }
            } else if (cd.mode == CM_GVAL || cd.mode == CM_GSEQ) {
                const uint32_t gbit = 1u << (cd.agg + (cd.mode == CM_GSEQ ? 16 : 0));
                const int j = select_marked_idx(tv.pm, ea.gplan + tv.in_base, gbit, last);
                if (j >= 0) {
                    const int pj = tv.pm[j] & kPmPosMask;
                    if (staged_valid(vw, pj)) { val = lds_fixed<W>(vals, pj); is_valid = true; }
                }
            } else if (GAGG && cd.mode == CM_GAGG) {
                fold_group_agg<false>(cd, tv.pm, ea.gagg + tv.in_base, vw, vals, last, &val, &is_valid, ea.err);
                if (!is_valid) val = 0;
            } else if (cd.mode == CM_KEY) {
                val = lds_fixed<W>(vals, tv.pm[last] & kPmPosMask); is_valid = true;
            } else if (cd.mode == CM_SEQ) {
                val = (uint64_t)ea.tmp_seq[result_index(tv, ob)]; is_valid = true;
            } else if (cd.mode == CM_KIND) {
                val = (uint8_t)ea.tmp_kind[result_index(tv, ob)]; is_valid = true;
            } else {
                fold_fixed<false>(cd, tv.pm, vw, vals, last, &val, &is_valid, ea.err);
                if (!is_valid) val = 0;
            }
            stg_fixed<W>(oc.data, tv.out_base + ob, val);
        }
        if (oc.validity != nullptr) put_validity_word(oc.validity, tv.out_base, wb, tv.n_out, is_valid);
    }
}

template <bool GAGG>
__device__ __forceinline__ void emit_decimal_column(const ColDesc &cd, const pg_out_column &oc, const TileView &tv,
                                                    const unsigned char *vals, const uint32_t *vw, const uint32_t *gagg,
                                                    int32_t *err) {
    const int tid = threadIdx.x, lane = tid & 31;
    for (int wb = (tid & ~31) - tv.o_shift; wb < tv.n_out; wb += kEmitThreads) {
        const int ob = wb + lane;
        bool is_valid = false;
        if (ob >= 0 && ob < tv.n_out) {
            uint64_t val = 0;
            const int last = tv.glast[ob];
            if (GAGG && cd.mode == CM_GAGG) fold_group_agg<true>(cd, tv.pm, gagg, vw, vals, last, &val, &is_valid, err);
            else fold_fixed<true>(cd, tv.pm, vw, vals, last, &val, &is_valid, err);
            stg_fixed<8>(oc.data, tv.out_base + ob, is_valid ? val : 0);
        }
        if (oc.validity != nullptr) put_validity_word(oc.validity, tv.out_base, wb, tv.n_out, is_valid);
    }
}

#ifdef PG_EMIT_TIMING
__device__ long long g_emit_ts[64 * 256];
#define TS(slot) do { if (tid == 0 && ts_on) g_emit_ts[(ts_tile) * 256 + (slot)] = clock64(); } while (0)
#else
#define TS(slot) do { } while (0)
#endif

struct PassEnt { ColDesc cd; pg_out_column oc; int32_t c, pad; };
constexpr int kPassCache = 64;

template <bool GAGG>
__global__ void __launch_bounds__(kEmitThreads, 2)
k_emit(EmitArgs ea) {
    extern __shared__ __align__(128) unsigned char smem[];
    __shared__ PassEnt s_pass[kPassCache];
    const int k = ea.k, tid = threadIdx.x, lane = tid & 31, warp = tid >> 5;
    const EmitLayout L = emit_layout(k);
    auto stage_vals = [&](int s) -> unsigned char * { return smem + (size_t)s * L.stage_bytes; };
    auto stage_vw = [&](int s) -> uint32_t * { return (uint32_t *)(smem + (size_t)s * L.stage_bytes + (size_t)L.rt * 8); };
    unsigned char *p = smem + kStages * L.stage_bytes;
    uint16_t *pm = (uint16_t *)p;              p += kTileMax * 2;
    uint16_t *glast = (uint16_t *)p;           p += kTileMax * 2;
    uint8_t *mrun = (uint8_t *)p;              p += kTileMax;
    int64_t *rstart = (int64_t *)p;            p += PG_MAX_RUNS * 8;
    const uint8_t **cdata = (const uint8_t **)p; p += kStages * PG_MAX_RUNS * 8;
    uint64_t *mbar = (uint64_t *)p;            p += kStages * 8;
    int64_t *s_i64 = (int64_t *)p;             p += 16;
    int *seg = (int *)p;                       p += (PG_MAX_RUNS + 1) * 4;
    int *seg_a = (int *)p;                     p += (PG_MAX_RUNS + 1) * 4;
    int *rr = (int *)p;                        p += (PG_MAX_RUNS + 1) * 4;
    int *ws = (int *)p;                        p += 34 * 4;
    int *s_i32 = (int *)p;                     p += 16;

    if (tid == 0) {
        s_i32[0] = atomicAdd(ea.tile_counter, 1);
        for (int s = 0; s < kStages; s++) mbar_init(&mbar[s], 1);
        mbar_fence_init();
    }
    __syncthreads();
    const int tile = s_i32[0];
    if (tid < ea.n_passes && tid < kPassCache) {
        const int c = ea.col_order[tid];
        s_pass[tid].c = c;
        s_pass[tid].cd = ea.cols[c];
        s_pass[tid].oc = ea.out_cols[c];
    }
#ifdef PG_EMIT_TIMING
    const bool ts_on = tile >= 2000 && tile < 2064;
    const int ts_tile = tile - 2000;
#endif
    TS(0);
    const int plan_a = 2 * tile, plan_end = min(plan_a + 2, ea.n_plan_tiles);
    if (warp == 0) {
        int64_t b0 = 0, bm = 0, b1 = 0;
        if (lane < k) {
            b0 = ea.bounds[(int64_t)plan_a * k + lane];
            bm = ea.bounds[(int64_t)(plan_a + 1) * k + lane];
            b1 = ea.bounds[(int64_t)plan_end * k + lane];
        }
        const int len = (int)(b1 - b0), len_a = (int)(bm - b0);
        const int rlen = lane < k ? (((int)(b0 & 31) + len + 1) + 31) & ~31 : 0;
        const int i_len = warp_scan_incl(len), i_a = warp_scan_incl(len_a), i_r = warp_scan_incl(rlen);
        if (lane < k) {
            rstart[lane] = b0;
            seg[lane] = i_len - len;
            seg_a[lane] = i_a - len_a;
            rr[lane] = i_r - rlen;
        }
        if (lane == 31) { seg[k] = i_len; seg_a[k] = i_a; rr[k] = i_r; }
    }
    __syncthreads();
    const int n = seg[k];
    const int n_vw = rr[k] >> 5;
    int64_t in_base = 0;
    for (int r = 0; r < k; r++) in_base += rstart[r];

    constexpr int VT = kTileMax / kEmitThreads;
    const int p0 = tid * VT, p1 = min(p0 + VT, n);
    int my = 0;
    uint32_t emit_bits = 0;
    uint16_t *spos = glast;
    uint8_t *srun = stage_vals(1);
    const int n_a = seg_a[k];
    for (int r = 0; r < k; r++) {
        const int len_a = seg_a[r + 1] - seg_a[r], len = seg[r + 1] - seg[r];
        const int p0r = rr[r] + (int)(rstart[r] & 31);
        const int sb0 = n_a + (seg[r] - seg_a[r]);
        for (int j = tid; j < len; j += kEmitThreads) {
            const int idx = j < len_a ? seg_a[r] + j : sb0 + (j - len_a);
            spos[idx] = (uint16_t)(p0r + j);
            srun[idx] = (uint8_t)r;
        }
    }
    __syncthreads();
    for (int i = p0; i < p1; i++) {
        uint16_t e = ea.plan[in_base + i];
        int slot = (e & kPlanSlotMask) + (i < n_a ? 0 : n_a);
        mrun[i] = srun[slot];
        uint32_t pos = spos[slot];
        uint32_t op = (e >> kPlanOpShift) & 3;
        pm[i] = (uint16_t)(pos | (op << kPmOpShift) | ((e & kPlanHead) ? kPmHead : 0));
        if ((e & kPlanHead) && (e & kPlanEmit)) { my++; emit_bits |= 1u << (i - p0); }
    }
    int n_out = 0;
    int o = block_scan_excl(my, ws, &n_out);
    for (int i = p0; i < p1; i++) {
        if (emit_bits & (1u << (i - p0))) {
            int e = i + 1;
            while (e < n && !(pm[e] & kPmHead)) e++;
            glast[o++] = (uint16_t)(e - 1);
        }
    }
    int vw_run = -1;
    int64_t vw_gword = 0;
    if (tid < n_vw) {
        int r = 0;
        while (r + 1 < k && (rr[r + 1] >> 5) <= tid) r++;
        vw_run = r;
        vw_gword = (rstart[r] >> 5) + (tid - (rr[r] >> 5));
        if (vw_gword > ((ea.run_rows[r] - 1) >> 5)) vw_run = -1;
    }
    __syncthreads();

    TileView tv;
    tv.pm = pm;
    tv.glast = glast;
    tv.n_out = n_out;
    tv.out_base = ea.row_base[plan_a];
    tv.o_shift = (int)(tv.out_base & 31);
    tv.in_base = in_base;
    tv.n_out_a = ea.tile_rows[plan_a];
    tv.seq_shift = n_a - tv.n_out_a;
    const int ncols = ea.n_passes;
    uint32_t phase = 0;

    auto col_staged = [&](const ColDesc &cd) { return cd.mode != CM_SEQ && cd.mode != CM_KIND; };
    auto pass_col = [&](int ci) -> int { return ci < kPassCache ? s_pass[ci].c : ea.col_order[ci]; };
    auto pass_desc = [&](int ci, int c) -> ColDesc { return ci < kPassCache ? s_pass[ci].cd : ea.cols[c]; };

    auto issue = [&](int c, const ColDesc &cd, int s) {
        if (!col_staged(cd)) return;
        asm volatile("fence.proxy.async.shared::cta;" ::: "memory");
        uint32_t bytes = 0;
        const unsigned char *src = nullptr;
        unsigned char *dst = nullptr;
        if (lane < k) {
            const int r = lane;
            const int len = seg[r + 1] - seg[r];
            const int64_t row0 = rstart[r] & ~(int64_t)31;
            const int head = (int)(rstart[r] & 31);
            if (cd.width > 0) {
                if (len > 0) {
                    bytes = (uint32_t)(((head + len) * cd.width + 15) & ~15);
                    src = (const unsigned char *)ea.ptrs.data[(int64_t)c * k + r] + row0 * cd.width;
                    dst = stage_vals(s) + (size_t)rr[r] * cd.width;
                }
            } else {
                if (len > 0) {
                    bytes = (uint32_t)(((head + len + 1) * 4 + 15) & ~15);
                    src = (const unsigned char *)(ea.ptrs.offsets[(int64_t)c * k + r] + row0);
                    dst = stage_vals(s) + (size_t)rr[r] * 4;
                }
                cdata[s * PG_MAX_RUNS + r] = (const uint8_t *)ea.ptrs.data[(int64_t)c * k + r];
            }
        }
        uint32_t total = bytes;
#pragma unroll
        for (int d = 16; d > 0; d >>= 1) total += __shfl_xor_sync(0xffffffffu, total, d);
        if (lane == 0) mbar_arrive_expect_tx(&mbar[s], total);
        __syncwarp();
        if (bytes) bulk_g2s(dst, src, bytes, &mbar[s]);
    };
    auto load_vw = [&](int c) -> uint32_t {
        if (vw_run < 0) return 0xffffffffu;
        const uint32_t *vp = ea.ptrs.validity[(int64_t)c * k + vw_run];
        return vp ? vp[vw_gword] : 0xffffffffu;
    };

    if (warp == 0 && ncols > 0) issue(pass_col(0), pass_desc(0, pass_col(0)), 0);
    if (tid < n_vw && ncols > 0) stage_vw(0)[tid] = load_vw(pass_col(0));
    __syncthreads();

    TS(1);
    for (int ci = 0; ci < ncols; ci++) {
        const int s = ci & 1;
        const int c = pass_col(ci);
        const int cn = ci + 1 < ncols ? pass_col(ci + 1) : -1;
        const ColDesc cd = pass_desc(ci, c);
        const pg_out_column oc = ci < kPassCache ? s_pass[ci].oc : ea.out_cols[c];
        if (warp == 0 && cn >= 0) issue(cn, pass_desc(ci + 1, cn), s ^ 1);
        uint32_t next_vw = (cn >= 0 && tid < n_vw) ? load_vw(cn) : 0;
        if (col_staged(cd)) {
            mbar_wait(&mbar[s], (phase >> s) & 1);
            phase ^= 1u << s;
        }
        const unsigned char *vals = stage_vals(s);
        const uint32_t *vw = stage_vw(s);

        if (cd.decimal) emit_decimal_column<GAGG>(cd, oc, tv, vals, vw, GAGG ? ea.gagg + tv.in_base : nullptr, ea.err);
        else if (cd.width == 8) emit_fixed_column<8, GAGG>(ea, cd, oc, tv, vals, vw);
        else if (cd.width == 4) emit_fixed_column<4, GAGG>(ea, cd, oc, tv, vals, vw);
        else if (cd.width == 1) emit_fixed_column<1, GAGG>(ea, cd, oc, tv, vals, vw);
        else if (cd.width == 2) emit_fixed_column<2, GAGG>(ea, cd, oc, tv, vals, vw);
        else {
            const int32_t *offs = (const int32_t *)vals;
            uint16_t *vsrc = (uint16_t *)(vals + (size_t)L.rt * 4);
            int *wpre = (int *)(vsrc + kTileMax);
            const uint8_t **wsrc = (const uint8_t **)(wpre + ((kEmitWarps * 33 + 1) & ~1));
            int *wend = (int *)(wsrc + kEmitWarps * 32);
            int64_t *wtot = (int64_t *)(wend + kEmitWarps * 32);
            static_assert(kTileMax * 2 + ((kEmitWarps * 33 + 1) & ~1) * 4 + kEmitWarps * 32 * (8 + 4) + kEmitWarps * 8 <=
                              (kTileMax + 64) * 4, "var-len scratch fits the upper half of a stage at k = 1");
            const uint8_t *const *cd_data = cdata + s * PG_MAX_RUNS;
            const int span = tv.o_shift + n_out;
            const int RW = (((span + kEmitWarps - 1) / kEmitWarps) + 31) & ~31;
            const int wbeg = -tv.o_shift + warp * RW;
            int64_t my_bytes = 0;
            for (int ob0 = wbeg; ob0 < wbeg + RW && ob0 < n_out; ob0 += 32) {
                const int ob = ob0 + lane;
                if (ob >= 0 && ob < n_out) {
                    const int last = glast[ob];
                    int src;
                    if (cd.mode == CM_KEY) src = last;
                    else if (cd.mode == CM_FOLD) src = fold_member_idx(cd, pm, mrun, vw, offs, cd_data, last, ea.err);
                    else if (cd.mode == CM_GVAL || cd.mode == CM_GSEQ) {
                        src = select_marked_idx(pm, ea.gplan + in_base,
                                                1u << (cd.agg + (cd.mode == CM_GSEQ ? 16 : 0)), last);
                        if (src >= 0 && !staged_valid(vw, pm[src] & kPmPosMask)) src = -1;
                    } else src = select_member_idx<GAGG>(pm, vw, last);
                    vsrc[ob] = src < 0 ? (uint16_t)0xFFFF : (uint16_t)src;
                    if (src >= 0) { int ps = pm[src] & kPmPosMask; my_bytes += offs[ps + 1] - offs[ps]; }
                }
            }
#pragma unroll
            for (int d = 16; d > 0; d >>= 1) my_bytes += __shfl_xor_sync(0xffffffffu, my_bytes, d);
            if (lane == 0) wtot[warp] = my_bytes;
            __syncthreads();
            if (ci < 60) TS(8 + 4 * ci + 0);
            uint64_t *state = ea.vl_state + (int64_t)cd.varlen_index * ea.n_tiles;
            if (warp == 0) {
                const int64_t x = lane < kEmitWarps ? wtot[lane] : 0;
                int64_t xi = x;
#pragma unroll
                for (int d = 1; d < kEmitWarps; d <<= 1) {
                    const int64_t y = __shfl_up_sync(0xffffffffu, xi, d);
                    if (lane >= d) xi += y;
                }
                const uint64_t tile_bytes = (uint64_t)__shfl_sync(0xffffffffu, xi, kEmitWarps - 1);
                if (lane < kEmitWarps) ws[lane] = (int)(xi - x);
                uint64_t excl = 0;
                if (lane == 0 && tile > 0) {
                    __threadfence();
                    atomicExch((unsigned long long *)&state[tile], kFlagAgg | (uint64_t)tile_bytes);
                }
                constexpr int kLook = 8;
                int t = tile - 1;
                while (t >= 0) {
                    uint64_t sv[kLook];
#pragma unroll
                    for (int q = 0; q < kLook; q++) {
                        const int idx = t - (lane * kLook + q);
                        sv[q] = idx >= 0 ? *((volatile uint64_t *)&state[idx]) : kFlagPrefix;
                    }
                    int lp = 32 * kLook;
#pragma unroll
                    for (int q = kLook - 1; q >= 0; q--) if ((unsigned)(sv[q] >> 62) == 2) lp = lane * kLook + q;
                    int first = lp;
#pragma unroll
                    for (int d = 16; d > 0; d >>= 1) first = min(first, __shfl_xor_sync(0xffffffffu, first, d));
                    bool inval = false;
                    uint64_t contrib = 0;
#pragma unroll
                    for (int q = 0; q < kLook; q++) {
                        if (lane * kLook + q <= first) {
                            if ((unsigned)(sv[q] >> 62) == 0) inval = true;
                            contrib += sv[q] & kValMask;
                        }
                    }
                    if (__any_sync(0xffffffffu, inval)) continue;
#pragma unroll
                    for (int d = 16; d > 0; d >>= 1) contrib += __shfl_xor_sync(0xffffffffu, contrib, d);
                    excl += contrib;
                    if (first < 32 * kLook) break;
                    t -= 32 * kLook;
                }
                if (lane == 0) {
                    __threadfence();
                    const uint64_t tot = excl + tile_bytes;
                    atomicExch((unsigned long long *)&state[tile], kFlagPrefix | tot);
                    const bool fits = tot <= 0x7fffffffull;
                    if (!fits) atomicCAS(ea.err, KERR_NONE, KERR_OFFSET_OVERFLOW);
                    s_i64[0] = fits ? (int64_t)excl : -1;
                    if (tile == ea.n_tiles - 1) {
                        ea.totals[1 + cd.varlen_index] = (int64_t)tot;
                        if (fits) oc.offsets[ea.totals[0]] = (int32_t)tot;
                    }
                }
            }
            __syncthreads();
            if (ci < 60) TS(8 + 4 * ci + 1);
            const int64_t byte_base = s_i64[0];
            uint8_t *dbase = (uint8_t *)oc.data + (byte_base < 0 ? 0 : byte_base);
            int carry = ws[warp];
            int *my_pre = wpre + warp * 33;
            int *my_end = wend + warp * 32;
            const uint8_t **my_src = wsrc + warp * 32;
            const int ob_end = byte_base < 0 ? wbeg : min(wbeg + RW, n_out);
            for (int ob0 = wbeg; ob0 < ob_end; ob0 += 32) {
                const int ob = ob0 + lane;
                const bool active = ob >= 0 && ob < n_out;
                int len = 0;
                const uint8_t *sp = nullptr;
                bool has = false;
                if (active) {
                    int src = vsrc[ob];
                    if (src != 0xFFFF) {
                        int ps = pm[src] & kPmPosMask;
                        int st = offs[ps];
                        len = offs[ps + 1] - st;
                        sp = cd_data[mrun[src]] + st;
                        has = true;
                    }
                }
                const int incl = warp_scan_incl(len);
                const int off = carry + incl - len;
                carry += __shfl_sync(0xffffffffu, incl, 31);
                if (active) oc.offsets[tv.out_base + ob] = (int32_t)(byte_base + off);
                if (oc.validity != nullptr) put_validity_word(oc.validity, tv.out_base, ob0, n_out, has);
                const unsigned pay = __ballot_sync(0xffffffffu, len > 0);
                const int n_pay = __popc(pay);
                if (len > 0) {
                    const int ci = __popc(pay & ((1u << lane) - 1));
                    my_pre[ci] = off;
                    my_end[ci] = off + len;
                    my_src[ci] = sp;
                }
                __syncwarp();
                for (int rg = 0; rg < n_pay; rg += 8) {
                    const int ra = rg + (lane >> 3), rb = ra + 4;
                    int a0 = 0, a1 = 0, b0 = 0, b1 = 0;
                    const uint8_t *pa = nullptr, *pb = nullptr;
                    if (ra < n_pay) { a0 = my_pre[ra]; a1 = my_end[ra]; pa = my_src[ra] - a0; }
                    if (rb < n_pay) { b0 = my_pre[rb]; b1 = my_end[rb]; pb = my_src[rb] - b0; }
                    const int64_t ia = (int64_t)a0 + (lane & 7), ib = (int64_t)b0 + (lane & 7);
                    uint8_t xa0 = 0, xa1 = 0, xa2 = 0, xb0 = 0, xb1 = 0, xb2 = 0;
                    if (ia < a1) xa0 = pa[ia];
                    if (ia + 8 < a1) xa1 = pa[ia + 8];
                    if (ia + 16 < a1) xa2 = pa[ia + 16];
                    if (ib < b1) xb0 = pb[ib];
                    if (ib + 8 < b1) xb1 = pb[ib + 8];
                    if (ib + 16 < b1) xb2 = pb[ib + 16];
                    if (ia < a1) dbase[ia] = xa0;
                    if (ia + 8 < a1) dbase[ia + 8] = xa1;
                    if (ia + 16 < a1) dbase[ia + 16] = xa2;
                    if (ib < b1) dbase[ib] = xb0;
                    if (ib + 8 < b1) dbase[ib + 8] = xb1;
                    if (ib + 16 < b1) dbase[ib + 16] = xb2;
                    for (int64_t b = ia + 24; b < a1; b += 8) dbase[b] = pa[b];
                    for (int64_t b = ib + 24; b < b1; b += 8) dbase[b] = pb[b];
                }
                __syncwarp();
            }
        }
        if (cn >= 0 && tid < n_vw) stage_vw(s ^ 1)[tid] = next_vw;
        __syncthreads();
        if (ci < 60) TS(8 + 4 * ci + 3);
    }
}

#ifdef PG_EMIT_TIMING
void emit_timing_dump() {
    static long long h[64 * 256];
    cudaDeviceSynchronize();
    cudaMemcpyFromSymbol(h, g_emit_ts, sizeof(h));
    double acc[256] = {0};
    int cntv[256] = {0};
    for (int t = 0; t < 64; t++)
        for (int sl = 1; sl < 256; sl++) {
            if (h[t * 256 + sl] == 0) continue;
            int pv = sl - 1;
            while (pv > 0 && h[t * 256 + pv] == 0) pv--;
            if (h[t * 256 + pv] == 0) continue;
            acc[sl] += (double)(h[t * 256 + sl] - h[t * 256 + pv]);
            cntv[sl]++;
        }
    fprintf(stderr, "[emit timing] cycles since previous slot (avg over tiles):");
    for (int sl = 1; sl < 256; sl++) if (cntv[sl]) fprintf(stderr, " %d:%.0f", sl, acc[sl] / cntv[sl]);
    fprintf(stderr, "\n");
    static long long z[64 * 256];
    cudaMemcpyToSymbol(g_emit_ts, z, sizeof(z));
}
#endif

static bool g_emit_attr = false;
void launch_emit(const EmitArgs &ea) {
    EmitLayout L = emit_layout(ea.k);
    if (!g_emit_attr) {
        cudaFuncSetAttribute(k_emit<false>, cudaFuncAttributeMaxDynamicSharedMemorySize, 200 * 1024);
        cudaFuncSetAttribute(k_emit<true>, cudaFuncAttributeMaxDynamicSharedMemorySize, 200 * 1024);
        g_emit_attr = true;
    }
    if (ea.gagg) k_emit<true><<<ea.n_tiles, kEmitThreads, L.total, ea.stream>>>(ea);
    else k_emit<false><<<ea.n_tiles, kEmitThreads, L.total, ea.stream>>>(ea);
#ifdef PG_EMIT_TIMING
    emit_timing_dump();
#endif
}

}
```

### paimon_b200/csrc/pg_internal.h

```cpp
#pragma once

#include <cuda_runtime.h>
#include <stdint.h>

#include <memory>
#include <mutex>
#include <string>
#include <unordered_map>
#include <utility>
#include <vector>

#include "paimon_gpu.h"
#include "range_reader.h"

namespace pg {

constexpr int kPlanTile = 2048;
constexpr int kTileMax = 2 * kPlanTile;
constexpr int kSampleStride = 16;
constexpr int kThreads = 256;
constexpr int kMaxCols = 256;

constexpr uint16_t kPlanSlotMask = 0x0FFF;
constexpr int kPlanOpShift = 12;
constexpr uint16_t kPlanEmit = 0x4000;
constexpr uint16_t kPlanHead = 0x8000;
enum : int { OP_NOOP = 0, OP_UPD = 1, OP_SET = 2, OP_RETRACT = 3 };

enum : int {
    KERR_NONE = 0,
    KERR_TILE_OVERFLOW = 1,
    KERR_PU_DELETE = 2,
    KERR_FIRST_ROW_RETRACT = 3,
    KERR_AGG_RETRACT = 4,
    KERR_OFFSET_OVERFLOW = 5,
    KERR_DIV_ZERO = 6,
    KERR_BAD_PAGE = 7,
    KERR_PQ_HEADER = 8,
    KERR_PQ_ENCODING = 9,
    KERR_PQ_NO_DICT = 10,
    KERR_PQ_ROWS = 11,
    KERR_PQ_DICT_ID = 12,
    KERR_PQ_LEVELS = 13,
    KERR_DEC_DIV_ZERO = 14,
    KERR_DEC_DIV_UNDEFINED = 15,
    KERR_DEC_NON_TERMINATING = 16
};

struct Schema {
    int n_key = 0, n_val = 0;
    std::vector<pg_field> key_fields, val_fields;
    int n_cols() const { return n_key + 2 + n_val; }
    pg_field field(int c) const {
        if (c < n_key) return key_fields[c];
        if (c == n_key) return pg_field{PG_INT64, 0};
        if (c == n_key + 1) return pg_field{PG_INT8, 0};
        return val_fields[c - n_key - 2];
    }
};

struct Spec {
    std::shared_ptr<const Schema> schema;
    int engine = 0, ignore_delete = 0, remove_record_on_delete = 0, drop_delete = 0;
    std::vector<int32_t> seq_fields;
    int seq_ascending = 1;
    std::vector<int32_t> agg;
    std::vector<uint8_t> ignore_retract;
    std::vector<int32_t> group_seq_start, group_seq_fields, field_group;
    std::vector<uint8_t> group_partial_delete;
    std::vector<uint8_t> read_fields;
    std::vector<int32_t> decimal;
    int n_groups() const { return group_seq_start.empty() ? 0 : (int)group_seq_start.size() - 1; }
};

struct DevColumn {
    const void *data = nullptr;
    const int32_t *offsets = nullptr;
    const uint8_t *validity = nullptr;
};

void *buf_take(size_t bytes, size_t *got);
void buf_give(void *p, size_t bytes);

class DeviceBuffer {
 public:
    DeviceBuffer() = default;
    explicit DeviceBuffer(size_t bytes) { p_ = buf_take(bytes, &n_); }
    DeviceBuffer(DeviceBuffer &&o) noexcept : p_(o.p_), n_(o.n_) { o.p_ = nullptr; o.n_ = 0; }
    DeviceBuffer &operator=(DeviceBuffer &&o) noexcept {
        std::swap(p_, o.p_);
        std::swap(n_, o.n_);
        return *this;
    }
    DeviceBuffer(const DeviceBuffer &) = delete;
    DeviceBuffer &operator=(const DeviceBuffer &) = delete;
    ~DeviceBuffer() { if (p_) buf_give(p_, n_); }
    unsigned char *get() const { return (unsigned char *)p_; }
    explicit operator bool() const { return p_ != nullptr; }

 private:
    void *p_ = nullptr;
    size_t n_ = 0;
};

inline size_t align256(size_t x) { return (x + 255) & ~(size_t)255; }

struct Run {
    Run(std::shared_ptr<const Schema> s, int64_t rows)
        : schema(std::move(s)), n_rows(rows), cols(schema->n_cols()), varlen_bytes(schema->n_cols(), 0),
          varlen_base(schema->n_cols(), 0) {}
    Run(const Run &) = delete;
    Run &operator=(const Run &) = delete;
    std::shared_ptr<const Schema> schema;
    int64_t n_rows;
    std::vector<DevColumn> cols;
    std::vector<int64_t> varlen_bytes;
    std::vector<int64_t> varlen_base;
    std::vector<DeviceBuffer> bufs;
    std::shared_ptr<const Run> source;
    int64_t bytes_h2d = 0;
};

struct Scratch {
    explicit Scratch(cudaStream_t s) : stream(s) {}
    ~Scratch() { if (!bufs.empty() || !runs.empty()) cudaStreamSynchronize(stream); }
    void *take(size_t bytes) {
        DeviceBuffer b(bytes ? bytes : 256);
        if (!b) return nullptr;
        bufs.push_back(std::move(b));
        return bufs.back().get();
    }
    cudaStream_t stream;
    std::vector<DeviceBuffer> bufs;
    std::vector<std::unique_ptr<Run>> runs;
};

pg_status oom(const char *who, const char *what, size_t bytes);

struct OutColumn {
    void *data = nullptr;
    int32_t *offsets = nullptr;
    uint32_t *validity = nullptr;
};

pg_status check_file_desc(const pg_file_desc &f);
pg_status check_section_args(uint64_t schema, const pg_file_desc *files, int n_files, int n_runs, const uint64_t *out_runs,
                             std::shared_ptr<const Schema> *s);
pg_status file_image(Scratch &scratch, const uint8_t *bytes, int64_t size, const char *who, const uint8_t **out);

struct RunBuilder {
    RunBuilder(std::shared_ptr<const Schema> s, int n_runs, Scratch &scratch, const char *who)
        : schema(std::move(s)), nc(schema->n_cols()), scratch(scratch), who(who), read(nc, 1), run_rows(n_runs, 0),
          missing((size_t)n_runs * nc, 0), with_rows((size_t)n_runs * nc, 0) {}
    pg_status read_columns(const uint8_t *read_cols, const char *const *names);
    pg_status add_file(int run, int64_t rows, const std::vector<std::string> &cols);
    int64_t place_file(int run, int64_t rows) {
        const int64_t row0 = run_rows[run];
        run_rows[run] += rows;
        return row0;
    }
    pg_status check_runs() const;
    pg_status alloc(const std::vector<uint8_t> &bitmap, const std::vector<uint8_t> &zero);
    pg_status alloc_payload(const std::vector<int64_t> &payload);
    void finish(uint64_t *out_runs, int64_t bytes_h2d, pg_section_info *info);

    const std::shared_ptr<const Schema> schema;
    const int nc;
    Scratch &scratch;
    const char *who;
    std::vector<uint8_t> read;
    const char *const *names = nullptr;
    std::vector<int64_t> run_rows;
    std::vector<std::vector<int>> file_col;
    std::vector<int64_t> file_row0;
    std::vector<uint8_t> missing;
    std::vector<uint8_t> with_rows;
    std::vector<OutColumn> out;
    int64_t decoded_bytes = 0;
};

struct SectionTimer {
    cudaEvent_t e0 = nullptr, e1 = nullptr;
    ~SectionTimer() {
        if (e0) cudaEventDestroy(e0);
        if (e1) cudaEventDestroy(e1);
    }
    float ms() const {
        float ms = 0;
        cudaEventElapsedTime(&ms, e0, e1);
        return ms;
    }
};

struct SectionFrame {
    SectionFrame(std::shared_ptr<const Schema> s, int n_runs, const char *who);
    pg_status start(const uint8_t *read_cols, const char *const *names);
    pg_status place(const pg_file_desc *files, int n_files);
    pg_status finish(const int32_t *d_err, uint64_t *out_runs, pg_section_info *info);

    const cudaStream_t stream;
    Scratch scratch;
    RunBuilder b;
    SectionTimer tm;
    int launches = 0;
    std::vector<const uint8_t *> d_file;
    int64_t file_bytes = 0, h2d = 0, page_bytes = 0;
};

template <typename T>
class Table {
 public:
    explicit Table(uint64_t tag) : tag_(tag << 56) {}
    uint64_t put(std::shared_ptr<T> p) {
        std::lock_guard<std::mutex> g(mu_);
        const uint64_t h = tag_ | next_++;
        map_[h] = std::move(p);
        return h;
    }
    std::shared_ptr<T> get(uint64_t h) {
        std::lock_guard<std::mutex> g(mu_);
        auto it = map_.find(h);
        return it == map_.end() ? nullptr : it->second;
    }
    std::shared_ptr<T> take(uint64_t h) {
        std::lock_guard<std::mutex> g(mu_);
        auto node = map_.extract(h);
        return node.empty() ? nullptr : std::move(node.mapped());
    }

 private:
    std::mutex mu_;
    std::unordered_map<uint64_t, std::shared_ptr<T>> map_;
    uint64_t next_ = 1;
    const uint64_t tag_;
};
extern Table<Schema> g_schemas;
extern Table<Run> g_runs;

pg_status ensure_device();
cudaStream_t copy_stream();
struct Merge;
struct BatchColumns {
    std::shared_ptr<const Schema> schema;
    std::vector<DevColumn> cols;
    int64_t n_rows = 0;
    std::shared_ptr<const Run> run;
    std::shared_ptr<Merge> merge;
};
pg_status batch_columns(uint64_t handle, BatchColumns *out);


struct ColDesc {
    int32_t type;
    int32_t width;
    int16_t nullable;
    int16_t retract;
    int32_t mode;
    int32_t agg;
    int32_t varlen_index;
    int32_t group;
    int32_t decimal;
};
static_assert(sizeof(ColDesc) == 32, "ColDesc is staged in shared memory by the emit kernel");
enum : int { CM_SELECT = 0, CM_FOLD = 1, CM_KEY = 2, CM_SEQ = 3, CM_KIND = 4, CM_GVAL = 5, CM_GSEQ = 6, CM_GAGG = 7 };
enum : int { RT_OK = 0, RT_IGNORE = 1, RT_ERROR = 2 };

struct MergeFlags {
    int32_t engine, ignore_delete, remove_record_on_delete, drop_delete;
};

struct KeyDesc {
    int32_t n_fields;
    int32_t exact;
    int32_t type[PG_MAX_KEY_FIELDS];
    int32_t width[PG_MAX_KEY_FIELDS];
};

struct KeySrc {
    const void *const *data;
    const int32_t *const *offsets;
};

inline int type_width(int t) {
    switch (t) {
        case PG_INT8: case PG_BOOL: return 1;
        case PG_INT16: return 2;
        case PG_INT32: case PG_FLOAT: return 4;
        case PG_INT64: case PG_DOUBLE: return 8;
        default: return 0;
    }
}
static bool type_ok(int t) { return t >= PG_INT8 && t <= PG_BINARY; }
inline bool is_varlen(int t) { return t == PG_STRING || t == PG_BINARY; }

void set_error(const std::string &msg);
pg_status fail(pg_status code, const std::string &msg);
pg_status kernel_error(int code, const char *who);

#define PG_CUDA(expr)                                                                      \
    do {                                                                                   \
        cudaError_t _e = (expr);                                                           \
        if (_e != cudaSuccess)                                                             \
            return pg::fail(PG_ERR_CUDA, std::string(#expr) + ": " + cudaGetErrorString(_e)); \
    } while (0)


struct LevelView {
    int64_t count[PG_MAX_RUNS];
    int64_t row0[PG_MAX_RUNS];
    int64_t stride;
};

struct MergeLaunch {
    int k;
    KeyDesc key;
    KeySrc ks;
    cudaStream_t stream;
    int32_t *err;
    const int *skip;
};

void launch_partition(const MergeLaunch &ml, const LevelView &lv, const uint64_t *splitter_keys,
                      const uint64_t *splitter_refs, int q, int n_tiles, int64_t *bounds);
void launch_key_lcp(const MergeLaunch &ml, const LevelView &lv0, int *skip);
void launch_merge_keys(const MergeLaunch &ml, const LevelView &lv, const int64_t *bounds, int n_tiles,
                       uint64_t *sorted_keys, uint64_t *sorted_refs);

struct ColPtrs {
    const void *const *data;
    const int32_t *const *offsets;
    const uint32_t *const *validity;
};

struct SeqFields {
    int32_t n;
    int32_t ascending;
    int32_t col[4];
    int32_t type[4];
    int32_t width[4];
};

struct SeqGroups {
    int32_t n;
    int32_t start[PG_MAX_SEQ_GROUPS + 1];
    int32_t col[PG_MAX_SEQ_GROUPS * 4];
    int32_t type[PG_MAX_SEQ_GROUPS * 4];
    int32_t width[PG_MAX_SEQ_GROUPS * 4];
    int32_t partial_delete[PG_MAX_SEQ_GROUPS];
};

struct PlanArgs {
    const int64_t *bounds;
    int n_tiles;
    SeqFields seq;
    ColPtrs ptrs;
    const int64_t *const *seq_ptrs;
    const int8_t *const *kind_ptrs;
    MergeFlags flags;
    uint16_t *plan;
    int32_t *tile_rows;
    int64_t *tmp_seq;
    int8_t *tmp_kind;
    const SeqGroups *groups;
    uint32_t *gplan;
    uint32_t *gagg;
};
void launch_plan(const MergeLaunch &ml, const PlanArgs &pa);

void launch_scan(cudaStream_t stream, const int32_t *tile_rows, int n_tiles, int64_t *row_base, int64_t *totals);

struct EmitArgs {
    const int64_t *bounds;
    int n_tiles;
    int n_plan_tiles;
    const int32_t *tile_rows;
    int k;
    const uint16_t *plan;
    const int64_t *row_base;
    const int64_t *tmp_seq;
    const int8_t *tmp_kind;
    const uint32_t *gplan;
    const uint32_t *gagg;
    const ColDesc *cols;
    const int32_t *col_order;
    int n_passes;
    const int32_t *varlen_cols;
    ColPtrs ptrs;
    const int64_t *run_rows;
    int n_cols;
    int n_varlen;
    const pg_out_column *out_cols;
    int64_t *totals;
    uint64_t *vl_state;
    int32_t *tile_counter;
    int32_t *err;
    cudaStream_t stream;
};
void launch_emit(const EmitArgs &ea);

pg_status small_h2d(void *dev_dst, const void *host_src, size_t n, cudaStream_t stream);

class SmallReads {
 public:
    explicit SmallReads(cudaStream_t s) : stream_(s) {}
    pg_status add(void *host_dst, const void *dev_src, size_t n);
    pg_status finish();

 private:
    struct Item { void *dst; size_t off, n; };
    cudaStream_t stream_;
    std::vector<Item> items_;
    size_t used_ = 0;
};

struct DeviceRanges : RangeReader {
    DeviceRanges(cudaStream_t s, const pg_file_desc *section, int n_files);
    void read(int file, uint64_t off, uint64_t n, uint8_t *dst) override;
    void flush() override;
    const pg_file_desc *section;
    std::vector<int> files;
    std::vector<uint64_t> sizes;
    SmallReads rb;
    pg_status st = PG_OK;
};

}
```

Measured before the change: 872.4 million.

## Split variable-length column emission into a separate kernel from fixed-width emit

Moves the variable-length column passes out of the main emit kernel into a new k_emit_varlen kernel that has its own thread count, shared-memory layout and tile counter. The shared tile prologue is factored into a helper that both kernels call. The fixed-width kernel drops the per-stage varlen data pointers and scratch. The goal is to stop varlen scratch and logic from inflating the fixed kernel's resources, at the cost of an extra launch and running the prologue twice when varlen columns exist. The int64 workload likely has no varlen columns, so on that path only the slimmer fixed kernel runs.

```diff
diff --git a/paimon_b200/csrc/api.cu b/paimon_b200/csrc/api.cu
--- a/paimon_b200/csrc/api.cu
+++ b/paimon_b200/csrc/api.cu
@@ -75,6 +75,7 @@
     int32_t *d_col_order = nullptr;
     int32_t *d_varlen_cols = nullptr;
     int n_passes = 0;
+    int n_varlen_passes = 0;
     const SeqGroups *d_groups = nullptr;
     bool has_group_aggs = false;
     pg_out_column *d_out_cols = nullptr;
@@ -588,6 +589,7 @@
         int32_t *vlc = (int32_t *)(host.data() + o_vlc);
         int n = 0;
         for (int c = 0; c < nc; c++) if (m->emit[c] && m->cols[c].width == 0) ord[n++] = c;
+        m->n_varlen_passes = n;
         for (int c = 0; c < nc; c++) if (m->emit[c] && m->cols[c].width != 0) ord[n++] = c;
         m->n_passes = n;
         for (int v = 0; v < nv; v++) vlc[v] = m->varlen_cols[v];
@@ -791,7 +793,7 @@
     PG_CUDA(talloc(sizeof(int64_t) * (size_t)T, (void **)&row_base));
     PG_CUDA(talloc(sizeof(uint64_t) * (size_t)T * std::max(nv, 1), (void **)&vl_state));
     PG_CUDA(cudaMemsetAsync(vl_state, 0, sizeof(uint64_t) * (size_t)T * std::max(nv, 1), sm));
-    PG_CUDA(cudaMemsetAsync(m->d_tile_counter, 0, sizeof(int32_t), sm));
+    PG_CUDA(cudaMemsetAsync(m->d_tile_counter, 0, 2 * sizeof(int32_t), sm));
 
     PlanArgs pa{};
     pa.bounds = bounds0;
@@ -886,6 +888,7 @@
     ea.cols = m->d_cols;
     ea.col_order = m->d_col_order;
     ea.n_passes = m->n_passes;
+    ea.n_varlen_passes = m->n_varlen_passes;
     ea.varlen_cols = m->d_varlen_cols;
     ea.ptrs = m->d_ptrs;
     ea.run_rows = m->d_run_rows;
@@ -895,11 +898,11 @@
     ea.totals = m->d_totals;
     ea.vl_state = vl_state;
     ea.tile_counter = m->d_tile_counter;
+    ea.varlen_tile_counter = m->d_tile_counter + 1;
     ea.err = m->d_err;
     ea.stream = sm;
     PG_CUDA(cudaEventRecord(m->ev[4], sm));
-    launch_emit(ea);
-    launches++;
+    launches += launch_emit(ea);
     PG_CUDA(cudaEventRecord(m->ev[3], sm));
     {
         SmallReads rb(sm);
diff --git a/paimon_b200/csrc/emit.cu b/paimon_b200/csrc/emit.cu
--- a/paimon_b200/csrc/emit.cu
+++ b/paimon_b200/csrc/emit.cu
@@ -6,7 +6,6 @@
 
 constexpr int kStages = 2;
 constexpr int kEmitThreads = 512;
-constexpr int kEmitWarps = kEmitThreads / 32;
 #define kFlagAgg (1ull << 62)
 #define kFlagPrefix (2ull << 62)
 #define kValMask ((1ull << 62) - 1)
@@ -25,7 +24,7 @@
     L.rt = kTileMax + 64 * k;
     L.stage_bytes = (((size_t)L.rt * 8 + (size_t)L.rt / 32 * 4) + 127) & ~(size_t)127;
     L.total = kStages * L.stage_bytes + (size_t)kTileMax * (2 + 2 + 1) + (PG_MAX_RUNS + 1) * 4 * 3 +
-              PG_MAX_RUNS * 8 + kStages * PG_MAX_RUNS * 8 + kStages * 8 + 34 * 4 + 64;
+              PG_MAX_RUNS * 8 + kStages * 8 + 34 * 4 + 64;
     return L;
 }
 
@@ -383,6 +382,126 @@
 struct PassEnt { ColDesc cd; pg_out_column oc; int32_t c, pad; };
 constexpr int kPassCache = 64;
 
+struct TileTables {
+    uint16_t *pm;
+    uint16_t *glast;
+    uint8_t *mrun;
+    int64_t *rstart;
+    int *seg, *seg_a, *rr;
+    int *ws;
+    uint8_t *scratch;
+};
+struct VwOwner { int run; int64_t gword; };
+
+template <int NT>
+__device__ __forceinline__ TileView tile_prologue(const EmitArgs &ea, int tile, const TileTables &tt, int *n_vw_out,
+                                                  VwOwner *vo) {
+    const int k = ea.k, tid = threadIdx.x, lane = tid & 31, warp = tid >> 5;
+    uint16_t *pm = tt.pm, *glast = tt.glast;
+    int64_t *rstart = tt.rstart;
+    int *seg = tt.seg, *seg_a = tt.seg_a, *rr = tt.rr;
+    const int plan_a = 2 * tile, plan_end = min(plan_a + 2, ea.n_plan_tiles);
+    if (warp == 0) {
+        int64_t b0 = 0, bm = 0, b1 = 0;
+        if (lane < k) {
+            b0 = ea.bounds[(int64_t)plan_a * k + lane];
+            bm = ea.bounds[(int64_t)(plan_a + 1) * k + lane];
+            b1 = ea.bounds[(int64_t)plan_end * k + lane];
+        }
+        const int len = (int)(b1 - b0), len_a = (int)(bm - b0);
+        const int rlen = lane < k ? (((int)(b0 & 31) + len + 1) + 31) & ~31 : 0;
+        const int i_len = warp_scan_incl(len), i_a = warp_scan_incl(len_a), i_r = warp_scan_incl(rlen);
+        if (lane < k) {
+            rstart[lane] = b0;
+            seg[lane] = i_len - len;
+            seg_a[lane] = i_a - len_a;
+            rr[lane] = i_r - rlen;
+        }
+        if (lane == 31) { seg[k] = i_len; seg_a[k] = i_a; rr[k] = i_r; }
+    }
+    __syncthreads();
+    const int n = seg[k];
+    const int n_vw = rr[k] >> 5;
+    int64_t in_base = 0;
+    for (int r = 0; r < k; r++) in_base += rstart[r];
+
+    constexpr int VT = (kTileMax + NT - 1) / NT;
+    static_assert(VT <= 32, "a thread's plan rows fit its 32-bit emit mask");
+    const int p0 = tid * VT, p1 = min(p0 + VT, n);
+    int my = 0;
+    uint32_t emit_bits = 0;
+    uint16_t *spos = glast;
+    uint8_t *srun = tt.scratch;
+    const int n_a = seg_a[k];
+    for (int r = 0; r < k; r++) {
+        const int len_a = seg_a[r + 1] - seg_a[r], len = seg[r + 1] - seg[r];
+        const int p0r = rr[r] + (int)(rstart[r] & 31);
+        const int sb0 = n_a + (seg[r] - seg_a[r]);
+        for (int j = tid; j < len; j += NT) {
+            const int idx = j < len_a ? seg_a[r] + j : sb0 + (j - len_a);
+            spos[idx] = (uint16_t)(p0r + j);
+            srun[idx] = (uint8_t)r;
+        }
+    }
+    __syncthreads();
+    for (int i = p0; i < p1; i++) {
+        uint16_t e = ea.plan[in_base + i];
+        int slot = (e & kPlanSlotMask) + (i < n_a ? 0 : n_a);
+        tt.mrun[i] = srun[slot];
+        uint32_t pos = spos[slot];
+        uint32_t op = (e >> kPlanOpShift) & 3;
+        pm[i] = (uint16_t)(pos | (op << kPmOpShift) | ((e & kPlanHead) ? kPmHead : 0));
+        if ((e & kPlanHead) && (e & kPlanEmit)) { my++; emit_bits |= 1u << (i - p0); }
+    }
+    int n_out = 0;
+    int o = block_scan_excl(my, tt.ws, &n_out);
+    for (int i = p0; i < p1; i++) {
+        if (emit_bits & (1u << (i - p0))) {
+            int e = i + 1;
+            while (e < n && !(pm[e] & kPmHead)) e++;
+            glast[o++] = (uint16_t)(e - 1);
+        }
+    }
+    vo->run = -1;
+    vo->gword = 0;
+    if (tid < n_vw) {
+        int r = 0;
+        while (r + 1 < k && (rr[r + 1] >> 5) <= tid) r++;
+        vo->run = r;
+        vo->gword = (rstart[r] >> 5) + (tid - (rr[r] >> 5));
+        if (vo->gword > ((ea.run_rows[r] - 1) >> 5)) vo->run = -1;
+    }
+    __syncthreads();
+    *n_vw_out = n_vw;
+
+    TileView tv;
+    tv.pm = pm;
+    tv.glast = glast;
+    tv.n_out = n_out;
+    tv.out_base = ea.row_base[plan_a];
+    tv.o_shift = (int)(tv.out_base & 31);
+    tv.in_base = in_base;
+    tv.n_out_a = ea.tile_rows[plan_a];
+    tv.seq_shift = n_a - tv.n_out_a;
+    return tv;
+}
+
+__device__ __forceinline__ uint32_t load_vw(const EmitArgs &ea, int c, const VwOwner &vo) {
+    if (vo.run < 0) return 0xffffffffu;
+    const uint32_t *vp = ea.ptrs.validity[(int64_t)c * ea.k + vo.run];
+    return vp ? vp[vo.gword] : 0xffffffffu;
+}
+
+__device__ __forceinline__ void cache_passes(const EmitArgs &ea, PassEnt *s_pass, int first, int n) {
+    const int tid = threadIdx.x;
+    if (tid < n && tid < kPassCache) {
+        const int c = ea.col_order[first + tid];
+        s_pass[tid].c = c;
+        s_pass[tid].cd = ea.cols[c];
+        s_pass[tid].oc = ea.out_cols[c];
+    }
+}
+
 template <bool GAGG>
 __global__ void __launch_bounds__(kEmitThreads, 2)
 k_emit(EmitArgs ea) {
@@ -393,18 +512,20 @@
     auto stage_vals = [&](int s) -> unsigned char * { return smem + (size_t)s * L.stage_bytes; };
     auto stage_vw = [&](int s) -> uint32_t * { return (uint32_t *)(smem + (size_t)s * L.stage_bytes + (size_t)L.rt * 8); };
     unsigned char *p = smem + kStages * L.stage_bytes;
-    uint16_t *pm = (uint16_t *)p;              p += kTileMax * 2;
-    uint16_t *glast = (uint16_t *)p;           p += kTileMax * 2;
-    uint8_t *mrun = (uint8_t *)p;              p += kTileMax;
-    int64_t *rstart = (int64_t *)p;            p += PG_MAX_RUNS * 8;
-    const uint8_t **cdata = (const uint8_t **)p; p += kStages * PG_MAX_RUNS * 8;
+    TileTables tt;
+    tt.pm = (uint16_t *)p;                     p += kTileMax * 2;
+    tt.glast = (uint16_t *)p;                  p += kTileMax * 2;
+    tt.mrun = (uint8_t *)p;                    p += kTileMax;
+    tt.rstart = (int64_t *)p;                  p += PG_MAX_RUNS * 8;
     uint64_t *mbar = (uint64_t *)p;            p += kStages * 8;
-    int64_t *s_i64 = (int64_t *)p;             p += 16;
-    int *seg = (int *)p;                       p += (PG_MAX_RUNS + 1) * 4;
-    int *seg_a = (int *)p;                     p += (PG_MAX_RUNS + 1) * 4;
-    int *rr = (int *)p;                        p += (PG_MAX_RUNS + 1) * 4;
-    int *ws = (int *)p;                        p += 34 * 4;
+    tt.seg = (int *)p;                         p += (PG_MAX_RUNS + 1) * 4;
+    tt.seg_a = (int *)p;                       p += (PG_MAX_RUNS + 1) * 4;
+    tt.rr = (int *)p;                          p += (PG_MAX_RUNS + 1) * 4;
+    tt.ws = (int *)p;                          p += 34 * 4;
     int *s_i32 = (int *)p;                     p += 16;
+    tt.scratch = stage_vals(1);
+    int *rr = tt.rr, *seg = tt.seg;
+    const int64_t *rstart = tt.rstart;
 
     if (tid == 0) {
         s_i32[0] = atomicAdd(ea.tile_counter, 1);
@@ -413,103 +534,20 @@
     }
     __syncthreads();
     const int tile = s_i32[0];
-    if (tid < ea.n_passes && tid < kPassCache) {
-        const int c = ea.col_order[tid];
-        s_pass[tid].c = c;
-        s_pass[tid].cd = ea.cols[c];
-        s_pass[tid].oc = ea.out_cols[c];
-    }
+    const int first = ea.n_varlen_passes, ncols = ea.n_passes - first;
+    cache_passes(ea, s_pass, first, ncols);
 #ifdef PG_EMIT_TIMING
     const bool ts_on = tile >= 2000 && tile < 2064;
     const int ts_tile = tile - 2000;
 #endif
     TS(0);
-    const int plan_a = 2 * tile, plan_end = min(plan_a + 2, ea.n_plan_tiles);
-    if (warp == 0) {
-        int64_t b0 = 0, bm = 0, b1 = 0;
-        if (lane < k) {
-            b0 = ea.bounds[(int64_t)plan_a * k + lane];
-            bm = ea.bounds[(int64_t)(plan_a + 1) * k + lane];
-            b1 = ea.bounds[(int64_t)plan_end * k + lane];
-        }
-        const int len = (int)(b1 - b0), len_a = (int)(bm - b0);
-        const int rlen = lane < k ? (((int)(b0 & 31) + len + 1) + 31) & ~31 : 0;
-        const int i_len = warp_scan_incl(len), i_a = warp_scan_incl(len_a), i_r = warp_scan_incl(rlen);
-        if (lane < k) {
-            rstart[lane] = b0;
-            seg[lane] = i_len - len;
-            seg_a[lane] = i_a - len_a;
-            rr[lane] = i_r - rlen;
-        }
-        if (lane == 31) { seg[k] = i_len; seg_a[k] = i_a; rr[k] = i_r; }
-    }
-    __syncthreads();
-    const int n = seg[k];
-    const int n_vw = rr[k] >> 5;
-    int64_t in_base = 0;
-    for (int r = 0; r < k; r++) in_base += rstart[r];
-
-    constexpr int VT = kTileMax / kEmitThreads;
-    const int p0 = tid * VT, p1 = min(p0 + VT, n);
-    int my = 0;
-    uint32_t emit_bits = 0;
-    uint16_t *spos = glast;
-    uint8_t *srun = stage_vals(1);
-    const int n_a = seg_a[k];
-    for (int r = 0; r < k; r++) {
-        const int len_a = seg_a[r + 1] - seg_a[r], len = seg[r + 1] - seg[r];
-        const int p0r = rr[r] + (int)(rstart[r] & 31);
-        const int sb0 = n_a + (seg[r] - seg_a[r]);
-        for (int j = tid; j < len; j += kEmitThreads) {
-            const int idx = j < len_a ? seg_a[r] + j : sb0 + (j - len_a);
-            spos[idx] = (uint16_t)(p0r + j);
-            srun[idx] = (uint8_t)r;
-        }
-    }
-    __syncthreads();
-    for (int i = p0; i < p1; i++) {
-        uint16_t e = ea.plan[in_base + i];
-        int slot = (e & kPlanSlotMask) + (i < n_a ? 0 : n_a);
-        mrun[i] = srun[slot];
-        uint32_t pos = spos[slot];
-        uint32_t op = (e >> kPlanOpShift) & 3;
-        pm[i] = (uint16_t)(pos | (op << kPmOpShift) | ((e & kPlanHead) ? kPmHead : 0));
-        if ((e & kPlanHead) && (e & kPlanEmit)) { my++; emit_bits |= 1u << (i - p0); }
-    }
-    int n_out = 0;
-    int o = block_scan_excl(my, ws, &n_out);
-    for (int i = p0; i < p1; i++) {
-        if (emit_bits & (1u << (i - p0))) {
-            int e = i + 1;
-            while (e < n && !(pm[e] & kPmHead)) e++;
-            glast[o++] = (uint16_t)(e - 1);
-        }
-    }
-    int vw_run = -1;
-    int64_t vw_gword = 0;
-    if (tid < n_vw) {
-        int r = 0;
-        while (r + 1 < k && (rr[r + 1] >> 5) <= tid) r++;
-        vw_run = r;
-        vw_gword = (rstart[r] >> 5) + (tid - (rr[r] >> 5));
-        if (vw_gword > ((ea.run_rows[r] - 1) >> 5)) vw_run = -1;
-    }
-    __syncthreads();
-
-    TileView tv;
-    tv.pm = pm;
-    tv.glast = glast;
-    tv.n_out = n_out;
-    tv.out_base = ea.row_base[plan_a];
-    tv.o_shift = (int)(tv.out_base & 31);
-    tv.in_base = in_base;
-    tv.n_out_a = ea.tile_rows[plan_a];
-    tv.seq_shift = n_a - tv.n_out_a;
-    const int ncols = ea.n_passes;
+    int n_vw;
+    VwOwner vo;
+    const TileView tv = tile_prologue<kEmitThreads>(ea, tile, tt, &n_vw, &vo);
     uint32_t phase = 0;
 
     auto col_staged = [&](const ColDesc &cd) { return cd.mode != CM_SEQ && cd.mode != CM_KIND; };
-    auto pass_col = [&](int ci) -> int { return ci < kPassCache ? s_pass[ci].c : ea.col_order[ci]; };
+    auto pass_col = [&](int ci) -> int { return ci < kPassCache ? s_pass[ci].c : ea.col_order[first + ci]; };
     auto pass_desc = [&](int ci, int c) -> ColDesc { return ci < kPassCache ? s_pass[ci].cd : ea.cols[c]; };
 
     auto issue = [&](int c, const ColDesc &cd, int s) {
@@ -521,21 +559,12 @@
         if (lane < k) {
             const int r = lane;
             const int len = seg[r + 1] - seg[r];
-            const int64_t row0 = rstart[r] & ~(int64_t)31;
-            const int head = (int)(rstart[r] & 31);
-            if (cd.width > 0) {
-                if (len > 0) {
-                    bytes = (uint32_t)(((head + len) * cd.width + 15) & ~15);
-                    src = (const unsigned char *)ea.ptrs.data[(int64_t)c * k + r] + row0 * cd.width;
-                    dst = stage_vals(s) + (size_t)rr[r] * cd.width;
-                }
-            } else {
-                if (len > 0) {
-                    bytes = (uint32_t)(((head + len + 1) * 4 + 15) & ~15);
-                    src = (const unsigned char *)(ea.ptrs.offsets[(int64_t)c * k + r] + row0);
-                    dst = stage_vals(s) + (size_t)rr[r] * 4;
-                }
-                cdata[s * PG_MAX_RUNS + r] = (const uint8_t *)ea.ptrs.data[(int64_t)c * k + r];
+            if (len > 0) {
+                const int64_t row0 = rstart[r] & ~(int64_t)31;
+                const int head = (int)(rstart[r] & 31);
+                bytes = (uint32_t)(((head + len) * cd.width + 15) & ~15);
+                src = (const unsigned char *)ea.ptrs.data[(int64_t)c * k + r] + row0 * cd.width;
+                dst = stage_vals(s) + (size_t)rr[r] * cd.width;
             }
         }
         uint32_t total = bytes;
@@ -545,14 +574,9 @@
         __syncwarp();
         if (bytes) bulk_g2s(dst, src, bytes, &mbar[s]);
     };
-    auto load_vw = [&](int c) -> uint32_t {
-        if (vw_run < 0) return 0xffffffffu;
-        const uint32_t *vp = ea.ptrs.validity[(int64_t)c * k + vw_run];
-        return vp ? vp[vw_gword] : 0xffffffffu;
-    };
 
     if (warp == 0 && ncols > 0) issue(pass_col(0), pass_desc(0, pass_col(0)), 0);
-    if (tid < n_vw && ncols > 0) stage_vw(0)[tid] = load_vw(pass_col(0));
+    if (tid < n_vw && ncols > 0) stage_vw(0)[tid] = load_vw(ea, pass_col(0), vo);
     __syncthreads();
 
     TS(1);
@@ -563,7 +587,7 @@
         const ColDesc cd = pass_desc(ci, c);
         const pg_out_column oc = ci < kPassCache ? s_pass[ci].oc : ea.out_cols[c];
         if (warp == 0 && cn >= 0) issue(cn, pass_desc(ci + 1, cn), s ^ 1);
-        uint32_t next_vw = (cn >= 0 && tid < n_vw) ? load_vw(cn) : 0;
+        uint32_t next_vw = (cn >= 0 && tid < n_vw) ? load_vw(ea, cn, vo) : 0;
         if (col_staged(cd)) {
             mbar_wait(&mbar[s], (phase >> s) & 1);
             phase ^= 1u << s;
@@ -576,165 +600,345 @@
         else if (cd.width == 4) emit_fixed_column<4, GAGG>(ea, cd, oc, tv, vals, vw);
         else if (cd.width == 1) emit_fixed_column<1, GAGG>(ea, cd, oc, tv, vals, vw);
         else if (cd.width == 2) emit_fixed_column<2, GAGG>(ea, cd, oc, tv, vals, vw);
-        else {
-            const int32_t *offs = (const int32_t *)vals;
-            uint16_t *vsrc = (uint16_t *)(vals + (size_t)L.rt * 4);
-            int *wpre = (int *)(vsrc + kTileMax);
-            const uint8_t **wsrc = (const uint8_t **)(wpre + ((kEmitWarps * 33 + 1) & ~1));
-            int *wend = (int *)(wsrc + kEmitWarps * 32);
-            int64_t *wtot = (int64_t *)(wend + kEmitWarps * 32);
-            static_assert(kTileMax * 2 + ((kEmitWarps * 33 + 1) & ~1) * 4 + kEmitWarps * 32 * (8 + 4) + kEmitWarps * 8 <=
-                              (kTileMax + 64) * 4, "var-len scratch fits the upper half of a stage at k = 1");
-            const uint8_t *const *cd_data = cdata + s * PG_MAX_RUNS;
-            const int span = tv.o_shift + n_out;
-            const int RW = (((span + kEmitWarps - 1) / kEmitWarps) + 31) & ~31;
-            const int wbeg = -tv.o_shift + warp * RW;
-            int64_t my_bytes = 0;
-            for (int ob0 = wbeg; ob0 < wbeg + RW && ob0 < n_out; ob0 += 32) {
-                const int ob = ob0 + lane;
-                if (ob >= 0 && ob < n_out) {
-                    const int last = glast[ob];
-                    int src;
-                    if (cd.mode == CM_KEY) src = last;
-                    else if (cd.mode == CM_FOLD) src = fold_member_idx(cd, pm, mrun, vw, offs, cd_data, last, ea.err);
-                    else if (cd.mode == CM_GVAL || cd.mode == CM_GSEQ) {
-                        src = select_marked_idx(pm, ea.gplan + in_base,
-                                                1u << (cd.agg + (cd.mode == CM_GSEQ ? 16 : 0)), last);
-                        if (src >= 0 && !staged_valid(vw, pm[src] & kPmPosMask)) src = -1;
-                    } else src = select_member_idx<GAGG>(pm, vw, last);
-                    vsrc[ob] = src < 0 ? (uint16_t)0xFFFF : (uint16_t)src;
-                    if (src >= 0) { int ps = pm[src] & kPmPosMask; my_bytes += offs[ps + 1] - offs[ps]; }
-                }
-            }
+        if (cn >= 0 && tid < n_vw) stage_vw(s ^ 1)[tid] = next_vw;
+        __syncthreads();
+        if (first + ci < 60) TS(8 + 4 * (first + ci) + 3);
+    }
+}
+
+constexpr int kVarThreads = 512;
+constexpr int kVarWarps = kVarThreads / 32;
+constexpr int kCopyChunks = 56;
+
+struct VarlenLayout {
+    int rt;
+    size_t stage_bytes;
+    size_t warp_bytes;
+    size_t total;
+};
+__host__ __device__ inline VarlenLayout varlen_layout(int k) {
+    VarlenLayout L;
+    L.rt = kTileMax + 64 * k;
+    L.stage_bytes = (((size_t)L.rt * 4 + (size_t)L.rt / 32 * 4) + 127) & ~(size_t)127;
+    L.warp_bytes = kCopyChunks * 16 + 32 * (4 + 4 + 8);
+    L.total = kStages * L.stage_bytes + kVarWarps * L.warp_bytes + (size_t)kTileMax * (2 + 2 + 2 + 1) +
+              PG_MAX_RUNS * 8 + kStages * PG_MAX_RUNS * 8 + kVarWarps * 8 + (PG_MAX_RUNS + 1) * 4 * 3 + kStages * 8 +
+              16 + 34 * 4 + 16 + 64;
+    return L;
+}
+
+__device__ __forceinline__ bool copy_range_words(uint4 *img, const uint8_t *sp, int len, uint8_t *dst,
+                                                 uint8_t *range_end) {
+    const int lane = threadIdx.x & 31;
+    const uintptr_t g0 = (uintptr_t)__shfl_sync(0xffffffffu, (unsigned long long)dst, 0);
+    const uintptr_t g1 = (uintptr_t)range_end;
+    const uintptr_t a0 = g0 & ~(uintptr_t)15;
+    const int nq = (int)((g1 - a0 + 15) >> 4);
+    if (nq > kCopyChunks) return false;
+    for (int q = lane; q < nq; q += 32) img[q] = make_uint4(0, 0, 0, 0);
+    __syncwarp();
+    if (len > 0) {
+        const int x = (int)((uintptr_t)dst - a0);
+        const uintptr_t t = (uintptr_t)sp - (uintptr_t)(x & 3);
+        const uint32_t sh = 8u * (uint32_t)(t & 3);
+        const uint32_t *sw = (const uint32_t *)(t & ~(uintptr_t)3);
+        const uintptr_t lo_ok = (uintptr_t)sp & ~(uintptr_t)15, hi_ok = ((uintptr_t)sp + len + 15) & ~(uintptr_t)15;
+        uint32_t *iw = (uint32_t *)img;
+        const int j0 = x >> 2, j1 = (x + len - 1) >> 2;
+        for (int j = j0; j <= j1; j += 4) {
+            uint32_t w[5];
 #pragma unroll
-            for (int d = 16; d > 0; d >>= 1) my_bytes += __shfl_xor_sync(0xffffffffu, my_bytes, d);
-            if (lane == 0) wtot[warp] = my_bytes;
-            __syncthreads();
-            if (ci < 60) TS(8 + 4 * ci + 0);
-            uint64_t *state = ea.vl_state + (int64_t)cd.varlen_index * ea.n_tiles;
-            if (warp == 0) {
-                const int64_t x = lane < kEmitWarps ? wtot[lane] : 0;
-                int64_t xi = x;
+            for (int u = 0; u < 5; u++) {
+                const uint32_t *a = sw + (j - j0) + u;
+                w[u] = ((uintptr_t)a >= lo_ok && (uintptr_t)a < hi_ok) ? __ldg(a) : 0u;
+            }
 #pragma unroll
-                for (int d = 1; d < kEmitWarps; d <<= 1) {
-                    const int64_t y = __shfl_up_sync(0xffffffffu, xi, d);
-                    if (lane >= d) xi += y;
-                }
-                const uint64_t tile_bytes = (uint64_t)__shfl_sync(0xffffffffu, xi, kEmitWarps - 1);
-                if (lane < kEmitWarps) ws[lane] = (int)(xi - x);
-                uint64_t excl = 0;
-                if (lane == 0 && tile > 0) {
-                    __threadfence();
-                    atomicExch((unsigned long long *)&state[tile], kFlagAgg | (uint64_t)tile_bytes);
-                }
-                constexpr int kLook = 8;
-                int t = tile - 1;
-                while (t >= 0) {
-                    uint64_t sv[kLook];
+            for (int u = 0; u < 4; u++) {
+                const int jj = j + u;
+                if (jj > j1) break;
+                const uint32_t v = __funnelshift_r(w[u], w[u + 1], sh);
+                const int bl = max(x - 4 * jj, 0), bh = min(x + len - 4 * jj, 4);
+                if (bl == 0 && bh == 4) iw[jj] = v;
+                else atomicOr(&iw[jj], v & ((0xffffffffu >> (32 - 8 * (bh - bl))) << (8 * bl)));
+            }
+        }
+    }
+    __syncwarp();
+    for (int q = lane; q < nq; q += 32) {
+        const uintptr_t a = a0 + 16 * (uintptr_t)q;
+        if (a >= g0 && a + 16 <= g1) *(uint4 *)a = img[q];
+    }
+    {
+        const int q = lane < 16 ? 0 : nq - 1;
+        const uintptr_t a = a0 + 16 * (uintptr_t)q;
+        const bool partial = a < g0 || a + 16 > g1;
+        const uintptr_t b = a + (lane & 15);
+        if (partial && (lane < 16 || nq > 1) && b >= g0 && b < g1) *(uint8_t *)b = ((const uint8_t *)img)[16 * q + (lane & 15)];
+    }
+    __syncwarp();
+    return true;
+}
+
+template <bool GAGG>
+__global__ void __launch_bounds__(kVarThreads, 2)
+k_emit_varlen(EmitArgs ea) {
+    extern __shared__ __align__(128) unsigned char smem[];
+    __shared__ PassEnt s_pass[kPassCache];
+    const int k = ea.k, tid = threadIdx.x, lane = tid & 31, warp = tid >> 5;
+    const VarlenLayout L = varlen_layout(k);
+    auto stage_offs = [&](int s) -> int32_t * { return (int32_t *)(smem + (size_t)s * L.stage_bytes); };
+    auto stage_vw = [&](int s) -> uint32_t * { return (uint32_t *)(smem + (size_t)s * L.stage_bytes + (size_t)L.rt * 4); };
+    unsigned char *p = smem + kStages * L.stage_bytes;
+    unsigned char *wbufs = p;                  p += kVarWarps * L.warp_bytes;
+    TileTables tt;
+    tt.pm = (uint16_t *)p;                     p += kTileMax * 2;
+    tt.glast = (uint16_t *)p;                  p += kTileMax * 2;
+    uint16_t *vsrc = (uint16_t *)p;            p += kTileMax * 2;
+    tt.mrun = (uint8_t *)p;                    p += kTileMax;
+    p = (unsigned char *)(((uintptr_t)p + 15) & ~(uintptr_t)15);
+    tt.rstart = (int64_t *)p;                  p += PG_MAX_RUNS * 8;
+    const uint8_t **cdata = (const uint8_t **)p; p += kStages * PG_MAX_RUNS * 8;
+    int64_t *wtot = (int64_t *)p;              p += kVarWarps * 8;
+    uint64_t *mbar = (uint64_t *)p;            p += kStages * 8;
+    int64_t *s_i64 = (int64_t *)p;             p += 16;
+    tt.seg = (int *)p;                         p += (PG_MAX_RUNS + 1) * 4;
+    tt.seg_a = (int *)p;                       p += (PG_MAX_RUNS + 1) * 4;
+    tt.rr = (int *)p;                          p += (PG_MAX_RUNS + 1) * 4;
+    tt.ws = (int *)p;                          p += 34 * 4;
+    int *s_i32 = (int *)p;                     p += 16;
+    tt.scratch = (uint8_t *)stage_offs(1);
+    const uint16_t *pm = tt.pm, *glast = tt.glast;
+    const uint8_t *mrun = tt.mrun;
+    const int *rr = tt.rr, *seg = tt.seg, *ws = tt.ws;
+    const int64_t *rstart = tt.rstart;
+
+    if (tid == 0) {
+        s_i32[0] = atomicAdd(ea.varlen_tile_counter, 1);
+        for (int s = 0; s < kStages; s++) mbar_init(&mbar[s], 1);
+        mbar_fence_init();
+    }
+    __syncthreads();
+    const int tile = s_i32[0];
+    const int ncols = ea.n_varlen_passes;
+    cache_passes(ea, s_pass, 0, ncols);
+#ifdef PG_EMIT_TIMING
+    const bool ts_on = tile >= 2000 && tile < 2064;
+    const int ts_tile = tile - 2000;
+#endif
+    TS(0);
+    int n_vw;
+    VwOwner vo;
+    const TileView tv = tile_prologue<kVarThreads>(ea, tile, tt, &n_vw, &vo);
+    const int n_out = tv.n_out;
+    uint32_t phase = 0;
+
+    auto pass_col = [&](int ci) -> int { return ci < kPassCache ? s_pass[ci].c : ea.col_order[ci]; };
+    auto issue = [&](int c, int s) {
+        asm volatile("fence.proxy.async.shared::cta;" ::: "memory");
+        uint32_t bytes = 0;
+        const unsigned char *src = nullptr;
+        unsigned char *dst = nullptr;
+        if (lane < k) {
+            const int r = lane;
+            const int len = seg[r + 1] - seg[r];
+            if (len > 0) {
+                const int64_t row0 = rstart[r] & ~(int64_t)31;
+                const int head = (int)(rstart[r] & 31);
+                bytes = (uint32_t)(((head + len + 1) * 4 + 15) & ~15);
+                src = (const unsigned char *)(ea.ptrs.offsets[(int64_t)c * k + r] + row0);
+                dst = (unsigned char *)(stage_offs(s) + rr[r]);
+            }
+            cdata[s * PG_MAX_RUNS + r] = (const uint8_t *)ea.ptrs.data[(int64_t)c * k + r];
+        }
+        uint32_t total = bytes;
 #pragma unroll
-                    for (int q = 0; q < kLook; q++) {
-                        const int idx = t - (lane * kLook + q);
-                        sv[q] = idx >= 0 ? *((volatile uint64_t *)&state[idx]) : kFlagPrefix;
-                    }
-                    int lp = 32 * kLook;
-#pragma unroll
-                    for (int q = kLook - 1; q >= 0; q--) if ((unsigned)(sv[q] >> 62) == 2) lp = lane * kLook + q;
-                    int first = lp;
-#pragma unroll
-                    for (int d = 16; d > 0; d >>= 1) first = min(first, __shfl_xor_sync(0xffffffffu, first, d));
-                    bool inval = false;
-                    uint64_t contrib = 0;
-#pragma unroll
-                    for (int q = 0; q < kLook; q++) {
-                        if (lane * kLook + q <= first) {
-                            if ((unsigned)(sv[q] >> 62) == 0) inval = true;
-                            contrib += sv[q] & kValMask;
-                        }
-                    }
-                    if (__any_sync(0xffffffffu, inval)) continue;
-#pragma unroll
-                    for (int d = 16; d > 0; d >>= 1) contrib += __shfl_xor_sync(0xffffffffu, contrib, d);
-                    excl += contrib;
-                    if (first < 32 * kLook) break;
-                    t -= 32 * kLook;
-                }
-                if (lane == 0) {
-                    __threadfence();
-                    const uint64_t tot = excl + tile_bytes;
-                    atomicExch((unsigned long long *)&state[tile], kFlagPrefix | tot);
-                    const bool fits = tot <= 0x7fffffffull;
-                    if (!fits) atomicCAS(ea.err, KERR_NONE, KERR_OFFSET_OVERFLOW);
-                    s_i64[0] = fits ? (int64_t)excl : -1;
-                    if (tile == ea.n_tiles - 1) {
-                        ea.totals[1 + cd.varlen_index] = (int64_t)tot;
-                        if (fits) oc.offsets[ea.totals[0]] = (int32_t)tot;
+        for (int d = 16; d > 0; d >>= 1) total += __shfl_xor_sync(0xffffffffu, total, d);
+        if (lane == 0) mbar_arrive_expect_tx(&mbar[s], total);
+        __syncwarp();
+        if (bytes) bulk_g2s(dst, src, bytes, &mbar[s]);
+    };
+
+    if (warp == 0 && ncols > 0) issue(pass_col(0), 0);
+    if (tid < n_vw && ncols > 0) stage_vw(0)[tid] = load_vw(ea, pass_col(0), vo);
+    __syncthreads();
+
+    const int span = tv.o_shift + n_out;
+    const int RW = (((span + kVarWarps - 1) / kVarWarps) + 31) & ~31;
+    const int wbeg = -tv.o_shift + warp * RW;
+    unsigned char *wbuf = wbufs + (size_t)warp * L.warp_bytes;
+
+    TS(1);
+    for (int ci = 0; ci < ncols; ci++) {
+        const int s = ci & 1;
+        const int c = pass_col(ci);
+        const int cn = ci + 1 < ncols ? pass_col(ci + 1) : -1;
+        const ColDesc cd = ci < kPassCache ? s_pass[ci].cd : ea.cols[c];
+        const pg_out_column oc = ci < kPassCache ? s_pass[ci].oc : ea.out_cols[c];
+        if (warp == 0 && cn >= 0) issue(cn, s ^ 1);
+        uint32_t next_vw = (cn >= 0 && tid < n_vw) ? load_vw(ea, cn, vo) : 0;
+        mbar_wait(&mbar[s], (phase >> s) & 1);
+        phase ^= 1u << s;
+        const int32_t *offs = stage_offs(s);
+        const uint32_t *vw = stage_vw(s);
+        const uint8_t *const *cd_data = cdata + s * PG_MAX_RUNS;
+
+        int64_t my_bytes = 0;
+        for (int ob0 = wbeg; ob0 < wbeg + RW && ob0 < n_out; ob0 += 32) {
+            const int ob = ob0 + lane;
+            if (ob >= 0 && ob < n_out) {
+                const int last = glast[ob];
+                int src;
+                if (cd.mode == CM_KEY) src = last;
+                else if (cd.mode == CM_FOLD) src = fold_member_idx(cd, pm, mrun, vw, offs, cd_data, last, ea.err);
+                else if (cd.mode == CM_GVAL || cd.mode == CM_GSEQ) {
+                    src = select_marked_idx(pm, ea.gplan + tv.in_base,
+                                            1u << (cd.agg + (cd.mode == CM_GSEQ ? 16 : 0)), last);
+                    if (src >= 0 && !staged_valid(vw, pm[src] & kPmPosMask)) src = -1;
+                } else src = select_member_idx<GAGG>(pm, vw, last);
+                vsrc[ob] = src < 0 ? (uint16_t)0xFFFF : (uint16_t)src;
+                if (src >= 0) {
+                    const int ps = pm[src] & kPmPosMask, st = offs[ps], len = offs[ps + 1] - st;
+                    my_bytes += len;
+                    if (len > 0) {
+                        const uint8_t *sp = cd_data[mrun[src]] + st;
+                        asm volatile("prefetch.global.L2 [%0];" ::"l"(sp));
+                        if (((uintptr_t)sp ^ ((uintptr_t)sp + len - 1)) >> 5)
+                            asm volatile("prefetch.global.L2 [%0];" ::"l"(sp + len - 1));
                     }
                 }
             }
-            __syncthreads();
-            if (ci < 60) TS(8 + 4 * ci + 1);
-            const int64_t byte_base = s_i64[0];
-            uint8_t *dbase = (uint8_t *)oc.data + (byte_base < 0 ? 0 : byte_base);
-            int carry = ws[warp];
-            int *my_pre = wpre + warp * 33;
-            int *my_end = wend + warp * 32;
-            const uint8_t **my_src = wsrc + warp * 32;
-            const int ob_end = byte_base < 0 ? wbeg : min(wbeg + RW, n_out);
-            for (int ob0 = wbeg; ob0 < ob_end; ob0 += 32) {
-                const int ob = ob0 + lane;
-                const bool active = ob >= 0 && ob < n_out;
-                int len = 0;
-                const uint8_t *sp = nullptr;
-                bool has = false;
-                if (active) {
-                    int src = vsrc[ob];
-                    if (src != 0xFFFF) {
-                        int ps = pm[src] & kPmPosMask;
-                        int st = offs[ps];
-                        len = offs[ps + 1] - st;
-                        sp = cd_data[mrun[src]] + st;
-                        has = true;
+        }
+#pragma unroll
+        for (int d = 16; d > 0; d >>= 1) my_bytes += __shfl_xor_sync(0xffffffffu, my_bytes, d);
+        if (lane == 0) wtot[warp] = my_bytes;
+        __syncthreads();
+        if (ci < 60) TS(8 + 4 * ci + 0);
+        uint64_t *state = ea.vl_state + (int64_t)cd.varlen_index * ea.n_tiles;
+        if (warp == 0) {
+            const int64_t x = lane < kVarWarps ? wtot[lane] : 0;
+            int64_t xi = x;
+#pragma unroll
+            for (int d = 1; d < kVarWarps; d <<= 1) {
+                const int64_t y = __shfl_up_sync(0xffffffffu, xi, d);
+                if (lane >= d) xi += y;
+            }
+            const uint64_t tile_bytes = (uint64_t)__shfl_sync(0xffffffffu, xi, kVarWarps - 1);
+            if (lane < kVarWarps) tt.ws[lane] = (int)(xi - x);
+            uint64_t excl = 0;
+            if (lane == 0 && tile > 0) {
+                __threadfence();
+                atomicExch((unsigned long long *)&state[tile], kFlagAgg | (uint64_t)tile_bytes);
+            }
+            constexpr int kLook = 4;
+            int t = tile - 1;
+            while (t >= 0) {
+                uint64_t sv[kLook];
+#pragma unroll
+                for (int q = 0; q < kLook; q++) {
+                    const int idx = t - (lane * kLook + q);
+                    sv[q] = idx >= 0 ? *((volatile uint64_t *)&state[idx]) : kFlagPrefix;
+                }
+                int lp = 32 * kLook;
+#pragma unroll
+                for (int q = kLook - 1; q >= 0; q--) if ((unsigned)(sv[q] >> 62) == 2) lp = lane * kLook + q;
+                int first = lp;
+#pragma unroll
+                for (int d = 16; d > 0; d >>= 1) first = min(first, __shfl_xor_sync(0xffffffffu, first, d));
+                bool inval = false;
+                uint64_t contrib = 0;
+#pragma unroll
+                for (int q = 0; q < kLook; q++) {
+                    if (lane * kLook + q <= first) {
+                        if ((unsigned)(sv[q] >> 62) == 0) inval = true;
+                        contrib += sv[q] & kValMask;
                     }
                 }
-                const int incl = warp_scan_incl(len);
-                const int off = carry + incl - len;
-                carry += __shfl_sync(0xffffffffu, incl, 31);
-                if (active) oc.offsets[tv.out_base + ob] = (int32_t)(byte_base + off);
-                if (oc.validity != nullptr) put_validity_word(oc.validity, tv.out_base, ob0, n_out, has);
-                const unsigned pay = __ballot_sync(0xffffffffu, len > 0);
-                const int n_pay = __popc(pay);
-                if (len > 0) {
-                    const int ci = __popc(pay & ((1u << lane) - 1));
-                    my_pre[ci] = off;
-                    my_end[ci] = off + len;
-                    my_src[ci] = sp;
+                if (__any_sync(0xffffffffu, inval)) continue;
+#pragma unroll
+                for (int d = 16; d > 0; d >>= 1) contrib += __shfl_xor_sync(0xffffffffu, contrib, d);
+                excl += contrib;
+                if (first < 32 * kLook) break;
+                t -= 32 * kLook;
+            }
+            if (lane == 0) {
+                __threadfence();
+                const uint64_t tot = excl + tile_bytes;
+                atomicExch((unsigned long long *)&state[tile], kFlagPrefix | tot);
+                const bool fits = tot <= 0x7fffffffull;
+                if (!fits) atomicCAS(ea.err, KERR_NONE, KERR_OFFSET_OVERFLOW);
+                s_i64[0] = fits ? (int64_t)excl : -1;
+                if (tile == ea.n_tiles - 1) {
+                    ea.totals[1 + cd.varlen_index] = (int64_t)tot;
+                    if (fits) oc.offsets[ea.totals[0]] = (int32_t)tot;
                 }
-                __syncwarp();
-                for (int rg = 0; rg < n_pay; rg += 8) {
-                    const int ra = rg + (lane >> 3), rb = ra + 4;
-                    int a0 = 0, a1 = 0, b0 = 0, b1 = 0;
-                    const uint8_t *pa = nullptr, *pb = nullptr;
-                    if (ra < n_pay) { a0 = my_pre[ra]; a1 = my_end[ra]; pa = my_src[ra] - a0; }
-                    if (rb < n_pay) { b0 = my_pre[rb]; b1 = my_end[rb]; pb = my_src[rb] - b0; }
-                    const int64_t ia = (int64_t)a0 + (lane & 7), ib = (int64_t)b0 + (lane & 7);
-                    uint8_t xa0 = 0, xa1 = 0, xa2 = 0, xb0 = 0, xb1 = 0, xb2 = 0;
-                    if (ia < a1) xa0 = pa[ia];
-                    if (ia + 8 < a1) xa1 = pa[ia + 8];
-                    if (ia + 16 < a1) xa2 = pa[ia + 16];
-                    if (ib < b1) xb0 = pb[ib];
-                    if (ib + 8 < b1) xb1 = pb[ib + 8];
-                    if (ib + 16 < b1) xb2 = pb[ib + 16];
-                    if (ia < a1) dbase[ia] = xa0;
-                    if (ia + 8 < a1) dbase[ia + 8] = xa1;
-                    if (ia + 16 < a1) dbase[ia + 16] = xa2;
-                    if (ib < b1) dbase[ib] = xb0;
-                    if (ib + 8 < b1) dbase[ib + 8] = xb1;
-                    if (ib + 16 < b1) dbase[ib + 16] = xb2;
-                    for (int64_t b = ia + 24; b < a1; b += 8) dbase[b] = pa[b];
-                    for (int64_t b = ib + 24; b < b1; b += 8) dbase[b] = pb[b];
+            }
+        }
+        __syncthreads();
+        if (ci < 60) TS(8 + 4 * ci + 1);
+        const int64_t byte_base = s_i64[0];
+        uint8_t *dbase = (uint8_t *)oc.data + (byte_base < 0 ? 0 : byte_base);
+        int carry = ws[warp];
+        int *my_pre = (int *)(wbuf + kCopyChunks * 16);
+        int *my_end = my_pre + 32;
+        const uint8_t **my_src = (const uint8_t **)(my_end + 32);
+        const int ob_end = byte_base < 0 ? wbeg : min(wbeg + RW, n_out);
+        for (int ob0 = wbeg; ob0 < ob_end; ob0 += 32) {
+            const int ob = ob0 + lane;
+            const bool active = ob >= 0 && ob < n_out;
+            int len = 0;
+            const uint8_t *sp = nullptr;
+            bool has = false;
+            if (active) {
+                int src = vsrc[ob];
+                if (src != 0xFFFF) {
+                    int ps = pm[src] & kPmPosMask;
+                    int st = offs[ps];
+                    len = offs[ps + 1] - st;
+                    sp = cd_data[mrun[src]] + st;
+                    has = true;
                 }
-                __syncwarp();
-            }
+            }
+            const int incl = warp_scan_incl(len);
+            const int off = carry + incl - len;
+            const int range = __shfl_sync(0xffffffffu, incl, 31);
+            carry += range;
+            if (active) oc.offsets[tv.out_base + ob] = (int32_t)(byte_base + off);
+            if (oc.validity != nullptr) put_validity_word(oc.validity, tv.out_base, ob0, n_out, has);
+            if (range == 0) continue;
+            if (copy_range_words((uint4 *)wbuf, sp, len, dbase + off, dbase + carry)) continue;
+            const unsigned pay = __ballot_sync(0xffffffffu, len > 0);
+            const int n_pay = __popc(pay);
+            if (len > 0) {
+                const int pi = __popc(pay & ((1u << lane) - 1));
+                my_pre[pi] = off;
+                my_end[pi] = off + len;
+                my_src[pi] = sp;
+            }
+            __syncwarp();
+            for (int rg = 0; rg < n_pay; rg += 8) {
+                const int ra = rg + (lane >> 3), rb = ra + 4;
+                int a0 = 0, a1 = 0, b0 = 0, b1 = 0;
+                const uint8_t *pa = nullptr, *pb = nullptr;
+                if (ra < n_pay) { a0 = my_pre[ra]; a1 = my_end[ra]; pa = my_src[ra] - a0; }
+                if (rb < n_pay) { b0 = my_pre[rb]; b1 = my_end[rb]; pb = my_src[rb] - b0; }
+                const int64_t ia = (int64_t)a0 + (lane & 7), ib = (int64_t)b0 + (lane & 7);
+                uint8_t xa0 = 0, xa1 = 0, xa2 = 0, xb0 = 0, xb1 = 0, xb2 = 0;
+                if (ia < a1) xa0 = pa[ia];
+                if (ia + 8 < a1) xa1 = pa[ia + 8];
+                if (ia + 16 < a1) xa2 = pa[ia + 16];
+                if (ib < b1) xb0 = pb[ib];
+                if (ib + 8 < b1) xb1 = pb[ib + 8];
+                if (ib + 16 < b1) xb2 = pb[ib + 16];
+                if (ia < a1) dbase[ia] = xa0;
+                if (ia + 8 < a1) dbase[ia + 8] = xa1;
+                if (ia + 16 < a1) dbase[ia + 16] = xa2;
+                if (ib < b1) dbase[ib] = xb0;
+                if (ib + 8 < b1) dbase[ib + 8] = xb1;
+                if (ib + 16 < b1) dbase[ib + 16] = xb2;
+                for (int64_t b = ia + 24; b < a1; b += 8) dbase[b] = pa[b];
+                for (int64_t b = ib + 24; b < b1; b += 8) dbase[b] = pb[b];
+            }
+            __syncwarp();
         }
         if (cn >= 0 && tid < n_vw) stage_vw(s ^ 1)[tid] = next_vw;
         __syncthreads();
@@ -743,7 +947,7 @@
 }
 
 #ifdef PG_EMIT_TIMING
-void emit_timing_dump() {
+void emit_timing_dump(const char *kernel) {
     static long long h[64 * 256];
     cudaDeviceSynchronize();
     cudaMemcpyFromSymbol(h, g_emit_ts, sizeof(h));
@@ -758,7 +962,7 @@
             acc[sl] += (double)(h[t * 256 + sl] - h[t * 256 + pv]);
             cntv[sl]++;
         }
-    fprintf(stderr, "[emit timing] cycles since previous slot (avg over tiles):");
+    fprintf(stderr, "[emit timing %s] cycles since previous slot (avg over tiles):", kernel);
     for (int sl = 1; sl < 256; sl++) if (cntv[sl]) fprintf(stderr, " %d:%.0f", sl, acc[sl] / cntv[sl]);
     fprintf(stderr, "\n");
     static long long z[64 * 256];
@@ -767,18 +971,32 @@
 #endif
 
 static bool g_emit_attr = false;
-void launch_emit(const EmitArgs &ea) {
-    EmitLayout L = emit_layout(ea.k);
+int launch_emit(const EmitArgs &ea) {
     if (!g_emit_attr) {
         cudaFuncSetAttribute(k_emit<false>, cudaFuncAttributeMaxDynamicSharedMemorySize, 200 * 1024);
         cudaFuncSetAttribute(k_emit<true>, cudaFuncAttributeMaxDynamicSharedMemorySize, 200 * 1024);
+        cudaFuncSetAttribute(k_emit_varlen<false>, cudaFuncAttributeMaxDynamicSharedMemorySize, 200 * 1024);
+        cudaFuncSetAttribute(k_emit_varlen<true>, cudaFuncAttributeMaxDynamicSharedMemorySize, 200 * 1024);
         g_emit_attr = true;
     }
+    int launches = 0;
+    if (ea.n_varlen_passes > 0) {
+        const VarlenLayout V = varlen_layout(ea.k);
+        if (ea.gagg) k_emit_varlen<true><<<ea.n_tiles, kVarThreads, V.total, ea.stream>>>(ea);
+        else k_emit_varlen<false><<<ea.n_tiles, kVarThreads, V.total, ea.stream>>>(ea);
+        launches++;
+#ifdef PG_EMIT_TIMING
+        emit_timing_dump("k_emit_varlen");
+#endif
+    }
+    const EmitLayout L = emit_layout(ea.k);
     if (ea.gagg) k_emit<true><<<ea.n_tiles, kEmitThreads, L.total, ea.stream>>>(ea);
     else k_emit<false><<<ea.n_tiles, kEmitThreads, L.total, ea.stream>>>(ea);
+    launches++;
 #ifdef PG_EMIT_TIMING
-    emit_timing_dump();
+    emit_timing_dump("k_emit");
 #endif
-}
-
-}
+    return launches;
+}
+
+}
diff --git a/paimon_b200/csrc/pg_internal.h b/paimon_b200/csrc/pg_internal.h
--- a/paimon_b200/csrc/pg_internal.h
+++ b/paimon_b200/csrc/pg_internal.h
@@ -384,6 +384,7 @@
     const ColDesc *cols;
     const int32_t *col_order;
     int n_passes;
+    int n_varlen_passes;
     const int32_t *varlen_cols;
     ColPtrs ptrs;
     const int64_t *run_rows;
@@ -393,10 +394,11 @@
     int64_t *totals;
     uint64_t *vl_state;
     int32_t *tile_counter;
+    int32_t *varlen_tile_counter;
     int32_t *err;
     cudaStream_t stream;
 };
-void launch_emit(const EmitArgs &ea);
+int launch_emit(const EmitArgs &ea);
 
 pg_status small_h2d(void *dev_dst, const void *host_src, size_t n, cudaStream_t stream);
 
diff --git a/profiles/emit_split.py b/profiles/emit_split.py
--- /dev/null
+++ b/profiles/emit_split.py
@@ -0,0 +1,165 @@
+import argparse
+import collections
+import json
+import os
+import re
+import subprocess
+import sys
+import tempfile
+
+ROOT = os.path.dirname(os.path.dirname(os.path.abspath(__file__)))
+sys.path.insert(0, ROOT)
+sys.path.insert(0, os.path.join(ROOT, "profiles"))
+os.environ.setdefault("PG_RUN_CACHE_BYTES", str(64 << 30))
+
+
+def c3_setup(rows):
+    import torch
+
+    import bench
+    from paimon_b200 import _native as N
+    from paimon_b200.sort_merge_reader import SortMergeReader
+
+    dev = torch.device("cuda", 0)
+    torch.cuda.set_device(dev)
+    w = bench.WORKLOADS["c3"]
+    schema = bench.make_schema("c3")
+    spec = bench.make_spec("c3", schema)
+    lib = N.init(0)
+    _, images, _, _ = bench.device_parquet_files("c3", schema, rows, dev, 100, lib)
+    files = [(img, r) for r, img in enumerate(images)]
+    rd = SortMergeReader([], spec, None, 0, schema=schema)
+    return schema, files, w["n_runs"], rd
+
+
+def merge_once(schema, files, n_runs, rd):
+    from paimon_b200.format import read_section
+    readers, _ = read_section(schema, files, n_runs, 0)
+    rd.rebind(readers)
+    rd.execute()
+    st = rd.stats()
+    for r in readers:
+        r.close()
+    rd.readers = []
+    return st
+
+
+def n_varlen_passes(schema):
+    from paimon_b200.types import is_varlen
+    return sum(1 for t in schema.physical_types() if is_varlen(t))
+
+
+def split_cycles(lines, nv):
+    out = collections.Counter()
+    per_col = collections.defaultdict(collections.Counter)
+    for line in lines:
+        for sl, cyc in re.findall(r" (\d+):(\d+)", line.split(":", 1)[1]):
+            sl, cyc = int(sl), float(cyc)
+            if sl == 1:
+                out["prologue"] += cyc
+                continue
+            if sl < 8:
+                continue
+            ci, part = divmod(sl - 8, 4)
+            if ci < nv:
+                name = {0: "varlen_pass1", 1: "varlen_lookback", 3: "varlen_pass2"}[part]
+            else:
+                name = "fixed"
+            out[name] += cyc
+            per_col[ci][name] += cyc
+    return out, per_col
+
+
+def run_timing(args):
+    schema, files, n_runs, rd = c3_setup(args.rows)
+    nv = n_varlen_passes(schema)
+    merge_once(schema, files, n_runs, rd)
+    res = []
+    for _ in range(args.reps):
+        with tempfile.TemporaryFile(mode="w+") as cap:
+            sys.stderr.flush()
+            saved = os.dup(2)
+            os.dup2(cap.fileno(), 2)
+            try:
+                merge_once(schema, files, n_runs, rd)
+            finally:
+                os.dup2(saved, 2)
+                os.close(saved)
+            cap.seek(0)
+            lines = [l for l in cap.read().splitlines() if l.startswith("[emit timing")]
+        tot, _ = split_cycles(lines, nv)
+        res.append(dict(tot))
+    rd.close()
+    print(json.dumps({"n_varlen_passes": nv, "reps": res}))
+
+
+def main():
+    ap = argparse.ArgumentParser()
+    ap.add_argument("--rows", type=int, default=None, help="total input rows (default: the bench's C3 size)")
+    ap.add_argument("--reps", type=int, default=3)
+    ap.add_argument("--timing-lib", default=None, help="a libpaimon_gpu.so built with -DPG_EMIT_TIMING")
+    ap.add_argument("--child-timing", action="store_true", help=argparse.SUPPRESS)
+    ap.add_argument("--out", default=os.path.join(tempfile.gettempdir(), "emit_split"))
+    args = ap.parse_args()
+    import bench
+    args.rows = args.rows or bench.WORKLOADS["c3"]["rows"]
+    if args.child_timing:
+        run_timing(args)
+        return
+
+    from decode_kernels import gpu_identity, short
+    summary = {"gpu": gpu_identity(0), "rows": args.rows}
+    if args.timing_lib:
+        env = dict(os.environ, PAIMON_GPU_LIB=os.path.abspath(args.timing_lib))
+        out = subprocess.run([sys.executable, os.path.abspath(__file__), "--child-timing", "--rows", str(args.rows),
+                              "--reps", str(args.reps)], env=env, capture_output=True, text=True, check=True).stdout
+        t = json.loads(out.strip().splitlines()[-1])
+        reps = t["reps"]
+        mean = {k: sum(r.get(k, 0.0) for r in reps) / len(reps) for k in sorted({k for r in reps for k in r})}
+        total = sum(mean.values())
+        varlen = sum(v for k, v in mean.items() if k.startswith("varlen"))
+        summary["cycles"] = {"n_varlen_passes": t["n_varlen_passes"], "per_tile": mean, "total": total,
+                             "varlen_share": varlen / total if total else None}
+
+    import torch
+    from torch.profiler import ProfilerActivity, profile
+    schema, files, n_runs, rd = c3_setup(args.rows)
+    for _ in range(2):
+        merge_once(schema, files, n_runs, rd)
+    torch.cuda.synchronize()
+    stats = []
+    with profile(activities=[ProfilerActivity.CUDA]) as prof:
+        for _ in range(args.reps):
+            stats.append(merge_once(schema, files, n_runs, rd))
+        torch.cuda.synchronize()
+    rd.close()
+    os.makedirs(args.out, exist_ok=True)
+    trace = os.path.join(args.out, "trace.pt.trace.json")
+    prof.export_chrome_trace(trace)
+    with open(trace) as f:
+        ev = json.load(f)["traceEvents"]
+    per = collections.defaultdict(lambda: {"launches": 0, "ms": 0.0})
+    for e in ev:
+        if e.get("cat") == "kernel" and "k_emit" in e.get("name", ""):
+            per[short(e["name"])]["launches"] += 1
+            per[short(e["name"])]["ms"] += float(e["dur"]) / 1e3
+    summary["kernels"] = {k: {"launches_per_merge": v["launches"] / args.reps, "ms_per_merge": v["ms"] / args.reps}
+                          for k, v in per.items()}
+    summary["ms_emit_events"] = [round(s.ms_emit, 3) for s in stats]
+    with open(os.path.join(args.out, "summary.json"), "w") as f:
+        json.dump(summary, f, indent=1)
+
+    print(json.dumps(summary["gpu"]), f"rows={args.rows}")
+    if "cycles" in summary:
+        c = summary["cycles"]
+        print(f"cycles per tile (avg over tiles 2000-2063, {c['n_varlen_passes']} var-len passes):")
+        for k, v in c["per_tile"].items():
+            print(f"  {k:<18}{v:>12.0f}{v / c['total']:>8.1%}")
+        print(f"  var-len share {c['varlen_share']:.1%}")
+    print("ms_emit (CUDA events):", summary["ms_emit_events"])
+    for k, v in summary["kernels"].items():
+        print(f"  {k:<28}{v['launches_per_merge']:>6g}{v['ms_per_merge']:>10.3f} ms")
+
+
+if __name__ == "__main__":
+    main()
```

Result: no change. 890.6 million, median of 6 (+2.1%).
